# Boese0601/Dyadic-Interaction-Modeling

Hardware: AMD Instinct MI355X
Metric: listener clips/sec (T=300, EMOCA-56) (higher is better)
Workload: dtype bf16; 1 GPU; C3: B=256/GPU synthetic dyad clips, T=300, SLMFT.forward(mode='val'): listener VQ encode + encoder + 299-step AR decode (top-k 52 sampling) + VQ decode; global_batch=256, seq_len=300, gather=tokens+coeffs, gather_bytes_per_rank=17452032

## Files before the change

### dyadic-interaction-modeling_amd/build.py

```python
import concurrent.futures
import os
import subprocess
import sys

HERE = os.path.dirname(os.path.abspath(__file__))
CSRC = os.path.join(HERE, "csrc")
OBJ = os.path.join(CSRC, "_obj")
LIB = os.path.join(HERE, "libdimx_hip.so")
SOURCES = ["gemm.hip", "gemm_x3.hip", "gemm256.hip", "norm.hip", "attention.hip", "attention_tr.hip", "mlp_fused.hip", "decode_attn.hip", "vq.hip", "elementwise.hip", "kv_prefill.hip", "chain.hip", "model.hip", "generate.hip", "ops.hip", "stream_attn.hip", "win_attn.hip", "stream.hip",
           "train_kernels.hip", "train_attn.hip", "train_vq.hip", "train.hip", "lstm.hip", "train_lstm.hip", "train_spk.hip", "fd_select.hip", "mesh_metrics.hip",
           "listener_metrics.hip", "kmeans_sid.hip", "seq_score.hip", "beam.hip", "consensus.hip", "retrieval.hip", "decode_attn_kv8.hip"]
HEADERS = ["common.hpp", "model.hpp", "stages.hpp", "train.hpp", "decode_attn_body.hpp", "sample_pick.hpp", "online_softmax_body.hpp", "frechet.hpp", "pick_gather.hpp", os.path.join("..", "..", "include", "dimx.h")]
FLAGS = ["--offload-arch=gfx950", "-O3", "-std=c++17", "-fPIC", "-Wall", "-Wno-unused-function",
         "-Wno-unused-variable", "-ffp-contract=on"]
SRC_FLAGS = {"attention_tr.hip": ["-fno-slp-vectorize"]}


def _hipcc():
    for c in (os.environ.get("HIPCC"), "/opt/rocm/bin/hipcc", "hipcc"):
        if c and (os.path.isabs(c) and os.path.exists(c) or not os.path.isabs(c)):
            return c
    return "hipcc"


def _file_hash(paths, extra=""):
    import hashlib
    hsh = hashlib.sha256(extra.encode())
    for f in paths:
        with open(f, "rb") as fh:
            hsh.update(os.path.basename(f).encode() + b"\0" + fh.read())
    return hsh.hexdigest()


def _compile(src):
    obj = os.path.join(OBJ, src.replace(".hip", ".o"))
    deps = [os.path.join(CSRC, src)] + [os.path.join(CSRC, h) for h in HEADERS]
    flags = FLAGS + SRC_FLAGS.get(src, [])
    want = _file_hash(deps, " ".join(flags))
    stamp = obj + ".srchash"
    if os.path.exists(obj) and os.path.exists(stamp):
        with open(stamp) as fh:
            if fh.read().strip() == want:
                return obj, False
    tmp = "%s.tmp.%d" % (obj, os.getpid())
    cmd = [_hipcc()] + flags + ["-c", os.path.join(CSRC, src), "-o", tmp]
    r = subprocess.run(cmd, capture_output=True, text=True)
    if r.returncode != 0:
        if os.path.exists(tmp):
            os.remove(tmp)
        raise RuntimeError("hipcc failed for %s:\n%s\n%s" % (src, r.stdout, r.stderr))
    if r.stderr.strip():
        sys.stderr.write(r.stderr)
    os.replace(tmp, obj)
    with open(stamp, "w") as fh:
        fh.write(want + "\n")
    return obj, True


def have_hipcc():
    import shutil
    c = _hipcc()
    return (os.path.isabs(c) and os.path.exists(c)) or shutil.which(c) is not None


STAMP = LIB + ".srchash"


def _src_hash():
    import hashlib
    hsh = hashlib.sha256((" ".join(FLAGS) + repr(sorted(SRC_FLAGS.items()))).encode())
    for f in SOURCES + HEADERS:
        with open(os.path.join(CSRC, f), "rb") as fh:
            hsh.update(f.encode() + b"\0" + fh.read())
    return hsh.hexdigest()


def stale():
    if not (os.path.exists(LIB) and os.path.exists(STAMP)):
        return True
    with open(STAMP) as fh:
        return fh.read().strip() != _src_hash()


def build(force=False):
    import fcntl
    os.makedirs(OBJ, exist_ok=True)
    with open(os.path.join(OBJ, ".lock"), "w") as lock:
        fcntl.flock(lock, fcntl.LOCK_EX)
        try:
            if not force and not stale():
                return LIB
            if force:
                for f in os.listdir(OBJ):
                    if f != ".lock" and os.path.isfile(os.path.join(OBJ, f)):
                        os.remove(os.path.join(OBJ, f))
            with concurrent.futures.ThreadPoolExecutor(max_workers=min(8, len(SOURCES))) as ex:
                res = list(ex.map(_compile, SOURCES))
            objs = [o for o, _ in res]
# ... 18 lines not shown
```

### dyadic-interaction-modeling_amd/csrc/common.hpp

```cpp
#pragma once
#include <hip/hip_runtime.h>
#include <stdint.h>
#include <stdio.h>
#include <string.h>
#include <string>

#include "../../include/dimx.h"

namespace dimx {

void set_error(const char* fmt, ...);
const char* get_error();

#define DIMX_HIP(expr)                                                                       \
    do {                                                                                     \
        hipError_t _e = (expr);                                                              \
        if (_e != hipSuccess) {                                                              \
            dimx::set_error("%s:%d: %s -> %s", __FILE__, __LINE__, #expr, hipGetErrorString(_e)); \
            return DIMX_ERR_HIP;                                                             \
        }                                                                                    \
    } while (0)

#define DIMX_REQUIRE(cond, code, ...)       \
    do {                                    \
// ... 193 lines not shown
    int kloop;
    int M, N, K;
    int conv_T;
    const int32_t* conv_lens;
    int conv_C;
    const float* bias;
    int act;
    const float* residual;
    int ldr;
    const float* rowadd;
    int rowadd_mode;
    float rowadd_scale;
    int rowadd_off, ld_rowadd;
    int rowadd_div;
    int rowT;
    OutSeg seg[3];
    int nseg, seg_width;
    int allow_splitk;
    int splitk;
    int force_simple;
    int cfg;
    int force_splitk;
    int out_slabs;
    long slab_stride;
    int stage_out;
    const float* ln_stats;
    const float* ln_colsum;
    int ln_C;
    unsigned* ln_err;
    int w_tiled;
    const void* w3;
    long w3_plane;
    int x3_decode;
    int vt_pack4;
};

void gemm_args_init(GemmArgs& a);
void gemm_set_plain_out(GemmArgs& a, void* C, int ldc);
int launch_gemm(const GemmArgs& a, hipStream_t s);
bool gemm256_eligible(const GemmArgs& a);
int launch_gemm256(const GemmArgs& a, hipStream_t s);
int launch_gemm256_segs(const GemmArgs& a, const OutSeg* segs, int nseg, int seg_width, hipStream_t s);
bool gemm_use_x3(const GemmArgs& a);
bool gemm_x3_plan(const GemmArgs& a, int* bn_out, int* sp_out);
int launch_gemm_x3(const GemmArgs& a, hipStream_t s);
int launch_split_x3(const float* w, void* planes, size_t n, hipStream_t s);
int gemm_plan_splits(const GemmArgs& a);

int launch_layernorm(int out_dtype, const float* x, void* y, const float* gamma, const float* beta, int M,
                     int C, hipStream_t s);
int launch_add_slabs_layernorm(int out_dtype, float* x, const float* slabs, int nslab, long slab_stride, void* y,
                               const float* gamma, int M, int C, hipStream_t s);
int launch_instnorm(int out_dtype, const float* x, void* y, const int32_t* lens, int B, int T, int C,
                    hipStream_t s);

struct AttnArgs {
    int dtype;
    const void *q, *k, *vt;
    void* o;
    long q_sb, q_st, q_sh;
    long k_sb, k_st, k_sh;
    long v_sb, v_sh, v_sd;
    int v_rows;
    long v_st;
    long o_sb, o_st, o_sh;
    int B, H, Lq, Lk, D;
    float scale;
    int causal;
    const int32_t* lens;
    const uint8_t* kmask;
    int kmask_ld;
    unsigned long long* kwords;
    size_t kwords_cap;
    int kwords_ready;
};
int launch_pack_key_words(const uint8_t* kmask, int kmask_ld, const int32_t* lens, int B, int Lk, unsigned long long* words, size_t cap,
                          hipStream_t s);
int launch_attention(const AttnArgs& a, hipStream_t s);
int launch_attention_tr(const AttnArgs& a, hipStream_t s);
size_t mlp_fused_packed_bytes(int C, int F);
int mlp_fused_pack(const float* w1, const float* b1, const float* w2, int C, int F, uint16_t* out);
int launch_mlp_fused(float* x, const void* packed, const float* b2, const float* ln_g, const float* ln_b, int M, int C, int F, int act,
                     hipStream_t s);

struct DecodeAttnArgs {
    int dtype;
    const void* q;
    int q_ld;
    int q_f32;
    int nslab;
    long slab_stride;
    int force_nsplit;
    int rows_per_clip;
    const void* knew;
    const void* vnew;
    int kv_ld;
    void* kcache;
    void* vcache;
    int Tmax;
    void* out;
    int o_ld;
    int B, H;
    const int32_t* step;
    int n_keys;
    const uint8_t* kmask;
    int kmask_ld;
    float scale;
    const void* tab;
    int tab_ld, tab_koff, tab_voff, tab_rows;
    const int32_t* hist;
    int hist_ld;
    int win, lookahead;
};
int launch_decode_attn(const DecodeAttnArgs& a, hipStream_t s);

struct Kv8AttnArgs {
    const float* q;
    int q_ld, nslab;
    long slab_stride;
    const uint8_t* kcodes;
    const float* kscale;
    const uint8_t* vcodes;
    const float* vscale;
    int Tmax;
    void* out;
    int out_dtype, o_ld;
    int B, H;
    int n_keys;
    const uint8_t* kmask;
    int kmask_ld;
    float scale;
    int force_nsplit;
    int win, lookahead;
    const int32_t* step;
};
int launch_decode_attn_kv8(const Kv8AttnArgs& a, hipStream_t s);
int launch_kv8_quant(int dtype, const void* cache, int B, int H, int Tp, int T, uint8_t* codes, float* scales, hipStream_t s);

int launch_vq_argmin(const float* z, int N, const float* Et , const float* ee ,
                     int32_t* idx, float* best_d, float* margin, hipStream_t s);

struct ChainGemmDesc {
    const void* W;
    int N, K, ldw;
    int cols, rows_pad, ncb, nkt;
};
struct ChainArgs {
    int B;
    ChainGemmDesc g1;
    const void* A1;
    int lda1;
    float* xr;
    float* x;
    int C;
    const float* slabs;
    int nslab;
    long slab_stride;
    void* y;
    const float* gamma;
    ChainGemmDesc g2;
    float* out2;
    int ld_out2;
    unsigned* counters;
    unsigned* seen;
    const int32_t* step;
    unsigned* err;
// ... 196 lines not shown
```

### dyadic-interaction-modeling_amd/csrc/generate.hip

```cpp
#include <stdlib.h>

#include "stages.hpp"

namespace dimx {

static void chain_desc(ChainGemmDesc& d, const Linear& L) { d.W = L.w; d.N = L.N; d.K = L.K; d.ldw = L.Kp; }

static bool gen_use_chain(dimx_handle h, int B, int S) {
    if (!h->use_chain || h->at != DIMX_BF16 || S != 1 || h->gen_groups > 1 || !h->chain_err_dev) return false;
    const DecGeom& dg = h->decg;
    ChainArgs c;
    memset(&c, 0, sizeof(c));
    c.B = B;
    c.C = dg.dim;
    const XAttn& sa = h->dec.self_[0];
    const XAttn& ca = h->dec.cross[0];
    chain_desc(c.g1, sa.out);
    c.lda1 = dg.heads * dg.dim_head;
    chain_desc(c.g2, ca.qkv);
    if (!chain_supported(c, h->cu_count)) return false;
    chain_desc(c.g2, h->dec.logits);
    c.g1.W = nullptr;
    return chain_supported(c, h->cu_count) && 3 * dg.depth + 1 <= kChainSites;
}
// ... 1007 lines not shown
                       const uint8_t* ctx_mask, const int32_t* lens, int B, int T, int beam_width, int32_t* tokens, double* scores,
                       int32_t* backptr, float* logits_out, void* beam_state, size_t beam_state_bytes, int flags, void* ws, size_t ws_bytes,
                       void* stream) {
    DIMX_REQUIRE(h, DIMX_ERR_ARG, "null handle");
    DIMX_NO_SESSION(h, "generate_beam");
    DIMX_REQUIRE(h->variant == 0, DIMX_ERR_ARG, "generate_beam: beam search is implemented for variant 0 (SLMFT) only; this handle is variant %d",
                 h->variant);
    DIMX_REQUIRE(!h->xwin_on, DIMX_ERR_ARG, "generate_beam: not available while the cross-attention window is on (dimx_set_cross_lookahead)");
    DIMX_REQUIRE(beam_width_supported(beam_width), DIMX_ERR_ARG, "generate_beam: beam_width %d not in {1,2,4,5,8,10}", beam_width);
    DIMX_REQUIRE(prompt && scores && T >= 2 && Pmax >= 1 && Pmax <= T - 1 && ld_prompt >= Pmax, DIMX_ERR_ARG,
                 "generate_beam: need scores, 1 <= Pmax <= T - 1 and ld_prompt >= Pmax (Pmax=%d T=%d ld_prompt=%d)", Pmax, T, ld_prompt);
    DIMX_REQUIRE(P0 >= 1 && P0 <= Pmax, DIMX_ERR_ARG, "generate_beam: need 1 <= P0 <= Pmax (P0=%d Pmax=%d)", P0, Pmax);
    DIMX_REQUIRE((flags & ~1) == 0, DIMX_ERR_ARG, "generate_beam: unknown flags 0x%x", flags);
    DIMX_REQUIRE(B >= 1 && T <= h->d.max_seq_len, DIMX_ERR_ARG, "B=%d T=%d out of range (T <= %d)", B, T, h->d.max_seq_len);
    const size_t R = (size_t)B * beam_width;
    DIMX_REQUIRE(beam_state && ((uintptr_t)beam_state % 8) == 0 && beam_state_bytes >= DIMX_BEAM_STATE_BYTES(B, beam_width), DIMX_ERR_ARG,
                 "generate_beam: the beam state needs %zu bytes, 8-byte aligned (DIMX_BEAM_STATE_BYTES); got %zu", (size_t)DIMX_BEAM_STATE_BYTES(B, beam_width),
                 beam_state_bytes);
    const int p0 = (flags & 1) ? 1 : P0;
    DIMX_REQUIRE(p0 == 1 || h->decg.dim_head == 64, DIMX_ERR_ARG, "generate_beam: the prefill needs 64-wide heads");
    const size_t need = workspace_bytes_prompt(h, B, T, beam_width, p0);
    DIMX_REQUIRE(ws_bytes >= need, DIMX_ERR_WORKSPACE, "generate_beam: workspace %zu < required %zu (dimx_workspace_bytes_prompt)", ws_bytes, need);
    BeamCall bm;
    bm.cum = (double*)beam_state;
    bm.parent = (int32_t*)((double*)beam_state + R);
    bm.backptr = backptr;
    bm.lens = lens;
    const GenRequest q{{prompt, ld_prompt, Pmax, prompt_len, p0 - 1}, ctx_mask, B, T, beam_width, 0.f, 0, nullptr, 0,
                       tokens, logits_out, ws, ws_bytes, (hipStream_t)stream, &bm};
    DIMX_TRY(generate_checked(h, q));
    DIMX_HIP(hipMemcpyAsync(scores, bm.cum, R * sizeof(double), hipMemcpyDeviceToDevice, (hipStream_t)stream));
    return DIMX_OK;
}

int dimx_set_sampler_filter(dimx_handle h, int kind, float a, float b) {
    DIMX_REQUIRE(h, DIMX_ERR_ARG, "null handle");
    DIMX_TRY(check_sampler_filter(kind, a, b));
    h->filter_kind = kind;
    h->filter_a = kind == DIMX_FILTER_TOP_K ? 0.f : a;
    h->filter_b = kind == DIMX_FILTER_TOP_A ? b : 0.f;
    return DIMX_OK;
}

int dimx_set_cross_lookahead(dimx_handle h, int on, int lookahead) {
    DIMX_REQUIRE(h, DIMX_ERR_ARG, "null handle");
    DIMX_NO_SESSION(h, "set_cross_lookahead");
    DIMX_REQUIRE(h->variant == 0, DIMX_ERR_ARG, "set_cross_lookahead: online generation is implemented for variant 0 (SLMFT) only; this handle is variant %d",
                 h->variant);
    h->xwin_on = on ? 1 : 0;
    h->xwin_lookahead = on ? lookahead : 0;
    return DIMX_OK;
}

int dimx_cross_lookahead(dimx_handle h, int* on, int* lookahead) {
    DIMX_REQUIRE(h, DIMX_ERR_ARG, "null handle");
    if (on) *on = h->xwin_on;
    if (lookahead) *lookahead = h->xwin_lookahead;
    return DIMX_OK;
}

size_t dimx_cross_kv8_bytes(dimx_handle h, int B, int T) { return kv8_bytes(h, B, T); }

int dimx_set_cross_kv8(dimx_handle h, void* buf, size_t bytes) {
    DIMX_REQUIRE(h, DIMX_ERR_ARG, "null handle");
    DIMX_NO_SESSION(h, "set_cross_kv8");
    DIMX_REQUIRE(h->variant == 0, DIMX_ERR_ARG, "set_cross_kv8: FP8 cross K/V is implemented for variant 0 (SLMFT) only; this handle is variant %d",
                 h->variant);
    DIMX_REQUIRE(buf == nullptr || (h->decg.dim_head == 64 && (uintptr_t)buf % 256 == 0), DIMX_ERR_ARG,
                 "set_cross_kv8: the buffer must be 256-byte aligned and the decoder's heads 64 wide");
    h->kv8_buf = buf;
    h->kv8_bytes = buf ? bytes : 0;
    return DIMX_OK;
}

int dimx_cross_kv8(dimx_handle h, void** buf, size_t* bytes) {
    DIMX_REQUIRE(h, DIMX_ERR_ARG, "null handle");
    if (buf) *buf = h->kv8_buf;
    if (bytes) *bytes = h->kv8_bytes;
    return DIMX_OK;
}

int dimx_chain_faults(dimx_handle h) { return h ? h->chain_faults : 0; }
int dimx_qkv0_table_builds(dimx_handle h) { return h ? h->qkv0_builds : 0; }
int dimx_kv0_table_generations(dimx_handle h) { return h ? h->kv0_generations : 0; }
int dimx_sample_head_generations(dimx_handle h) { return h ? h->sample_head_generations : 0; }

int dimx_debug_chain_fault(dimx_handle h, int n_calls) {
    DIMX_REQUIRE(h && n_calls >= 0, DIMX_ERR_ARG, "debug_chain_fault: bad argument");
    h->chain_fault_inject = n_calls;
    h->graph_valid = false;
    return DIMX_OK;
}

}
```

### dyadic-interaction-modeling_amd/csrc/model.hip

```cpp
#include <stdarg.h>
#include <stdlib.h>
#include <set>

#include "stages.hpp"

namespace dimx {

static thread_local char g_err[1024] = "";
void set_error(const char* fmt, ...) {
    va_list ap;
    va_start(ap, fmt);
    vsnprintf(g_err, sizeof(g_err), fmt, ap);
    va_end(ap);
}
const char* get_error() { return g_err; }

static std::string vq_prefix(int which) { return which == 0 ? "speaker_vq." : "listener_vq."; }

struct KeySpec {
    std::string name;
    std::vector<int64_t> shape;
};

static void vq_keys(const dimx_dims& d, int which, std::vector<KeySpec>& out) {
// ... 232 lines not shown
        }
        row += rows;
    }
    void* p;
    if (c->at == DIMX_BF16) {
        std::vector<uint16_t> wb(w.size());
        for (size_t i = 0; i < w.size(); ++i) wb[i] = host_f32_to_bf16(w[i]);
        DIMX_TRY(dev_upload(c, wb.data(), wb.size() * 2, &p));
    } else {
        DIMX_TRY(dev_upload(c, w.data(), w.size() * 4, &p));
    }
    out->w = p;
    out->N = N;
    out->K = K;
    out->Kp = Kp;
    out->bias = nullptr;
    if (!bias.empty()) DIMX_TRY(upload_f32(c, bias, &out->bias));
    return DIMX_OK;
}

static int make_x3(dimx_ctx* c, Linear* L) {
    static const bool off = getenv("DIMX_NO_X3") != nullptr;
    L->w3 = nullptr;
    if (off || c->at != DIMX_F32 || !L->w || L->Kp % 32 != 0) return DIMX_OK;
    const size_t n = (size_t)L->N * L->Kp;
    void* p = nullptr;
    DIMX_HIP(hipMalloc(&p, 3 * n * 2));
    c->dev_allocs.push_back(p);
    DIMX_TRY(launch_split_x3((const float*)L->w, p, n, nullptr));
    DIMX_HIP(hipStreamSynchronize(nullptr));
    L->w3 = p;
    return DIMX_OK;
}

static int pack_linear_scaled(dimx_ctx* c, const std::string& wname, const std::string& gname, const std::string& bias,
                              Linear* out, const float** colsum) {
    auto wi = c->host.find(wname), gi = c->host.find(gname);
    DIMX_REQUIRE(wi != c->host.end() && gi != c->host.end(), DIMX_ERR_WEIGHT, "missing weight %s / %s", wname.c_str(), gname.c_str());
    const int N = (int)wi->second.shape[0], K = (int)wi->second.shape[1];
    DIMX_REQUIRE((int)gi->second.data.size() == K && K % 64 == 0, DIMX_ERR_WEIGHT, "%s: gamma / K mismatch", wname.c_str());
    std::vector<uint16_t> wb((size_t)N * K);
    std::vector<float> cs(N);
    for (int n = 0; n < N; ++n) {
        double acc = 0.0;
        for (int k = 0; k < K; ++k) {
            const uint16_t b = host_f32_to_bf16(wi->second.data[(size_t)n * K + k] * gi->second.data[k]);
            wb[(size_t)n * K + k] = b;
            const uint32_t u = (uint32_t)b << 16;
            float f;
            memcpy(&f, &u, 4);
            acc += f;
        }
        cs[n] = (float)acc;
    }
    void *p, *q;
    DIMX_TRY(dev_upload(c, wb.data(), wb.size() * 2, &p));
    DIMX_TRY(dev_upload(c, cs.data(), cs.size() * 4, &q));
    out->w = p;
    out->N = N;
    out->K = K;
    out->Kp = K;
    out->bias = nullptr;
    if (!bias.empty()) DIMX_TRY(upload_f32(c, bias, &out->bias));
    *colsum = (const float*)q;
    return DIMX_OK;
}

static int pack_mlp(dimx_ctx* c, const std::string& w1, const std::string& b1, const std::string& w2, const void** out) {
    *out = nullptr;
    if (c->at != DIMX_BF16) return DIMX_OK;
    auto i1 = c->host.find(w1), ib = c->host.find(b1), i2 = c->host.find(w2);
    DIMX_REQUIRE(i1 != c->host.end() && ib != c->host.end() && i2 != c->host.end(), DIMX_ERR_WEIGHT, "missing weight %s", w1.c_str());
    const int F = (int)i1->second.shape[0], C = (int)i1->second.shape[1];
    const size_t bytes = mlp_fused_packed_bytes(C, F);
    if (bytes == 0 || (int)i2->second.shape[0] != C || (int)i2->second.shape[1] != F) return DIMX_OK;
    std::vector<uint16_t> img(bytes / 2);
    DIMX_TRY(mlp_fused_pack(i1->second.data.data(), ib->second.data.data(), i2->second.data.data(), C, F, img.data()));
    void* p;
    DIMX_TRY(dev_upload(c, img.data(), bytes, &p));
    *out = p;
    return DIMX_OK;
}

static int pack_vq(dimx_ctx* c, int which) {
    VQNet& v = c->vq[which];
    const VQGeom& vg = c->vqg[which];
    const std::string p = vq_prefix(which), e = p + "encoder.", d = p + "decoder.";
    DIMX_TRY(pack_linear(c, {e + "vertice_mapping.0.weight"}, e + "vertice_mapping.0.bias", false, &v.vm));
    DIMX_TRY(pack_linear(c, {e + "squasher.0.0.weight"}, e + "squasher.0.0.bias", true, &v.conv));
    DIMX_TRY(pack_linear(c, {e + "encoder_linear_embedding.net.weight"}, e + "encoder_linear_embedding.net.bias", false, &v.le));
    DIMX_TRY(pack_linear(c, {e + "encoder_linear_embedding_post.net.weight"}, e + "encoder_linear_embedding_post.net.bias", false, &v.post));
    if (vg.has_decoder) {
        DIMX_TRY(pack_linear(c, {d + "decoder_linear_embedding_pre.net.weight"}, d + "decoder_linear_embedding_pre.net.bias", false, &v.pre));
        DIMX_TRY(pack_linear(c, {d + "expander.0.0.weight"}, d + "expander.0.0.bias", true, &v.dconv));
        DIMX_TRY(pack_linear(c, {d + "decoder_linear_embedding.net.weight"}, d + "decoder_linear_embedding.net.bias", false, &v.dle));
        DIMX_TRY(pack_linear(c, {d + "vertice_map_reverse.weight"}, "", false, &v.rev));
    }
    for (int s = 0; s < (vg.has_decoder ? 2 : 1); ++s) {
        const std::string pre = s == 0 ? e + "encoder_transformer." : d + "decoder_transformer.";
        VQBlock* blk = s == 0 ? v.enc : v.dec;
        for (int i = 0; i < vg.layers; ++i) {
            const std::string a = pre + "net." + std::to_string(2 * i) + ".fn.";
            const std::string m = pre + "net." + std::to_string(2 * i + 1) + ".fn.";
            DIMX_TRY(upload_f32(c, a + "norm.weight", &blk[i].ln1_g));
            DIMX_TRY(upload_f32(c, a + "norm.bias", &blk[i].ln1_b));
            DIMX_TRY(pack_linear(c, {a + "fn.to_qkv.weight"}, "", false, &blk[i].qkv));
            DIMX_TRY(pack_linear(c, {a + "fn.to_out.weight"}, a + "fn.to_out.bias", false, &blk[i].out));
            DIMX_TRY(upload_f32(c, m + "norm.weight", &blk[i].ln2_g));
            DIMX_TRY(upload_f32(c, m + "norm.bias", &blk[i].ln2_b));
            DIMX_TRY(pack_linear(c, {m + "fn.l1.weight"}, m + "fn.l1.bias", false, &blk[i].l1));
            DIMX_TRY(pack_linear(c, {m + "fn.l2.weight"}, m + "fn.l2.bias", false, &blk[i].l2));
            DIMX_TRY(pack_mlp(c, m + "fn.l1.weight", m + "fn.l1.bias", m + "fn.l2.weight", &blk[i].mlp));
        }
    }
    DIMX_TRY(upload_f32(c, e + "encoder_pos_embedding.pe", &v.pe_enc));
    if (vg.has_decoder) DIMX_TRY(upload_f32(c, d + "decoder_pos_embedding.pe", &v.pe_dec));
    DIMX_TRY(upload_f32(c, p + "quantize.embedding.weight", &v.E));
    const HostTensor& E = c->host[p + "quantize.embedding.weight"];
    const int ne = vg.n_embed, zd = vg.zdim;
    std::vector<float> Et((size_t)zd * ne), ee(ne);
    for (int j = 0; j < ne; ++j) {
        float s = 0.f;
        for (int k = 0; k < zd; ++k) {
            const float x = E.data[(size_t)j * zd + k];
            Et[(size_t)k * ne + j] = x;
            s = fmaf(x, x, s);
        }
        ee[j] = s;
    }
    void* pp;
    DIMX_TRY(dev_upload(c, Et.data(), Et.size() * 4, &pp));
    v.Et = (const float*)pp;
    DIMX_TRY(dev_upload(c, ee.data(), ee.size() * 4, &pp));
    v.ee = (const float*)pp;
    return DIMX_OK;
}

static int pack_xattn(dimx_ctx* c, const std::string& p, bool cross, XAttn* a) {
    DIMX_TRY(upload_f32(c, p + "0.0.weight", &a->ln_g));
    if (cross) {
        DIMX_TRY(pack_linear(c, {p + "1.to_q.weight"}, "", false, &a->qkv));
    } else {
        DIMX_TRY(pack_linear(c, {p + "1.to_q.weight", p + "1.to_k.weight", p + "1.to_v.weight"}, "", false, &a->qkv));
    }
    DIMX_TRY(pack_linear(c, {p + "1.to_out.weight"}, "", false, &a->out));
    return DIMX_OK;
}
static int pack_xff(dimx_ctx* c, const std::string& p, XFF* f) {
    DIMX_TRY(upload_f32(c, p + "0.0.weight", &f->ln_g));
    DIMX_TRY(pack_linear(c, {p + "1.ff.0.0.weight"}, p + "1.ff.0.0.bias", false, &f->f1));
    DIMX_TRY(pack_linear(c, {p + "1.ff.2.weight"}, p + "1.ff.2.bias", false, &f->f2));
    DIMX_TRY(pack_mlp(c, p + "1.ff.0.0.weight", p + "1.ff.0.0.bias", p + "1.ff.2.weight", &f->mlp));
    return DIMX_OK;
}
static int pack_xenc(dimx_ctx* c, const std::string& pre, XEnc* e) {
    DIMX_TRY(pack_linear(c, {pre + "project_in.weight"}, c->host.count(pre + "project_in.bias") ? pre + "project_in.bias" : "", false,
                         &e->proj_in));
    DIMX_TRY(upload_f32(c, pre + "pos_emb.emb.weight", &e->pos_emb));
    for (int i = 0; i < c->encg[0].depth; ++i) {
        DIMX_TRY(pack_xattn(c, xl(pre, 2 * i), false, &e->attn[i]));
        DIMX_TRY(pack_xff(c, xl(pre, 2 * i + 1), &e->ff[i]));
    }
    DIMX_TRY(upload_f32(c, pre + "attn_layers.final_norm.weight", &e->final_g));
    return DIMX_OK;
}

static void free_packed(dimx_ctx* c) {
    for (void* p : c->dev_allocs) (void)hipFree(p);
    c->dev_allocs.clear();
    c->packed_mask = 0;
    ++c->dec_epoch;
}


static std::vector<KeySpec> comp_keys(const dimx_dims& d, int comp) {
    std::vector<KeySpec> k;
    if (comp == COMP_MESH) {
        mesh_keys(d, k);
        return k;
    }
    if (d.variant == 1) {
        if (comp == COMP_VQ0) legacy_speaker_vq_keys(d, k);
        if (comp == COMP_VQ1) vq_keys(d, 1, k);
        if (comp == COMP_ENC) xenc_keys(d, "generator.encoder.", (int64_t)d.spk_face_quan_num * d.vq_zdim, k);
        if (comp == COMP_DEC) {
            xdec_keys(d, "generator.decoder.net.", k);
            k.push_back({"generator.decoder.net.pos_emb.emb.weight", {d.max_seq_len, d.dim + d.dim_a}});
        }
        return k;
    }
    if (comp == COMP_VQ0) vq_keys(d, 0, k);
    if (comp == COMP_VQ1) vq_keys(d, 1, k);
    if (comp == COMP_ENC) {
        xenc_keys(d, "encoder_s.", d.dim_in, k);
        xenc_keys(d, "encoder_joint.", d.dim, k);
        k.push_back({"patch_embed_s", {1, 1, d.dim_in}});
        k.push_back({"patch_embed_dec_s", {1, 1, d.dim}});
        k.push_back({"norm_s.weight", {d.dim}});
        k.push_back({"norm_s.bias", {d.dim}});
        if (d.variant == 2) slm_extra_keys(d, k, 1);
    }
    if (comp == COMP_DEC) {
        xdec_keys(d, "decoder_joint.net.", k);
        if (d.variant == 2) slm_extra_keys(d, k, 2);
    }
    return k;
}

static int ensure_packed(dimx_ctx* c, int need) {
    if ((c->packed_mask & need) == need) return DIMX_OK;
    DIMX_HIP(hipSetDevice(c->device));
    for (int comp = 1; comp <= COMP_MESH; comp <<= 1) {
        if (!(need & comp) || (c->packed_mask & comp)) continue;
        int missing = 0;
        std::string first;
        for (const auto& k : comp_keys(c->d, comp))
            if (!c->host.count(k.name)) {
                if (!missing) first = k.name;
                ++missing;
            }
        DIMX_REQUIRE(missing == 0, DIMX_ERR_WEIGHT, "%d weights of this stage not loaded (first: %s)", missing,
                     first.c_str());
        if (comp == COMP_VQ0) DIMX_TRY(pack_vq(c, 0));
        if (comp == COMP_VQ1) DIMX_TRY(pack_vq(c, 1));
        if (comp == COMP_ENC && c->variant == 1) {
            DIMX_TRY(pack_xenc(c, "generator.encoder.", &c->enc_s));
// ... 108 lines not shown
    return at == DIMX_BF16 && D <= 64;
}

static void set_qkv_out(GemmArgs& g, void* q, void* k, void* vt, int T, int H, int D, int Tp, bool rowv = false) {
    const int segw = H * D;
    g.rowT = T;
    g.nseg = 3;
    g.seg_width = segw;
    for (int i = 0; i < (rowv ? 3 : 2); ++i) {
        g.seg[i].ptr = i == 0 ? q : (i == 1 ? k : vt);
        g.seg[i].sb = (long)T * segw;
        g.seg[i].st = segw;
        g.seg[i].sh = D;
        g.seg[i].sd = 1;
        g.seg[i].D = D;
    }
    if (rowv) return;
    g.seg[2].ptr = vt;
    g.seg[2].sb = (long)H * D * Tp;
    g.seg[2].sh = (long)D * Tp;
    g.seg[2].sd = Tp;
    g.seg[2].st = 1;
    g.seg[2].D = D;
}

void set_attn_packed(AttnArgs& a, int dtype, const void* q, const void* k, const void* vt, void* o, int B,
                            int H, int Lq, int Lk, int D, int Tp_k, bool rowv) {
    memset(&a, 0, sizeof(a));
    const int segw = H * D;
    a.dtype = dtype;
    a.q = q;
    a.k = k;
    a.vt = vt;
    a.o = o;
    a.q_sb = (long)Lq * segw;
    a.q_st = segw;
    a.q_sh = D;
    a.k_sb = (long)Lk * segw;
    a.k_st = segw;
    a.k_sh = D;
    a.v_sb = (long)H * D * Tp_k;
    a.v_sh = (long)D * Tp_k;
    a.v_sd = Tp_k;
    if (rowv) {
        a.v_rows = 1;
        a.v_sb = (long)Lk * segw;
        a.v_st = segw;
        a.v_sh = D;
    }
    a.o_sb = (long)Lq * segw;
    a.o_st = segw;
    a.o_sh = D;
    a.B = B;
    a.H = H;
    a.Lq = Lq;
    a.Lk = Lk;
    a.D = D;
}


int linear(const dimx_ctx* c, const void* A, int lda, const Linear& L, int M, int out_dtype, void* out, int ldo, hipStream_t st, int act,
           const float* residual) {
    GemmArgs g;
    gemm_lin(c, A, lda, L, M, g);
    g.out_dtype = out_dtype; g.act = act;
    g.residual = residual; g.ldr = residual ? ldo : 0;
    gemm_set_plain_out(g, out, ldo);
    return launch_gemm(g, st);
}
int residual_linear(const dimx_ctx* c, const void* A, int lda, const Linear& L, int M, float* h, int ld, hipStream_t st) {
    return linear(c, A, lda, L, M, DIMX_F32, h, ld, st, ACT_NONE, h);
}

constexpr int kFusedMlpMinRows = 8192;

int ff_sublayer(const dimx_ctx* c, const BlockBufs& b, const float* ln_g, const float* ln_b, const Linear& f1,
                       const Linear& f2, const void* mlp, int act, int M, int C, hipStream_t st) {
    if (mlp && M >= kFusedMlpMinRows) return launch_mlp_fused(b.h, mlp, f2.bias, ln_g, ln_b, M, C, f1.N, act, st);
    DIMX_TRY(launch_layernorm(c->at, b.h, b.y, ln_g, ln_b, M, C, st));
    DIMX_TRY(linear(c, b.y, C, f1, M, c->at, b.f, f1.N, st, act));
    return residual_linear(c, b.f, f1.N, f2, M, b.h, C, st);
}

int self_attn_qkv(const dimx_ctx* c, const BlockBufs& b, const float* ln_g, const float* ln_b, const Linear& qkv, int B,
                         int T, int C, int heads, int D, AttnArgs& a, hipStream_t st) {
    const bool rowv = qkv_row_v(c->at, D);
    DIMX_TRY(launch_layernorm(c->at, b.h, b.y, ln_g, ln_b, B * T, C, st));
    GemmArgs g;
    gemm_lin(c, b.y, C, qkv, B * T, g);
    g.out_dtype = c->at;
    set_qkv_out(g, b.q, b.k, b.vt, T, heads, D, tpad(T), rowv);
    DIMX_TRY(launch_gemm(g, st));
    set_attn_packed(a, c->at, b.q, b.k, b.vt, b.o, B, heads, T, T, D, tpad(T), rowv);
    return DIMX_OK;
}

int attn_out(const dimx_ctx* c, const BlockBufs& b, AttnArgs& a, const Linear& out, int C, hipStream_t st) {
    a.kwords = b.kw; a.kwords_cap = b.kw_cap;
    DIMX_TRY(launch_attention(a, st));
    return residual_linear(c, b.o, a.H * a.D, out, a.B * a.Lq, b.h, C, st);
}

int cross_attn_sublayer(const dimx_ctx* c, const BlockBufs& b, const XAttn& x, AttnArgs& a, const uint8_t* ctx_mask, int C,
                               hipStream_t st, const float* v_rows) {
    const int M = a.B * a.Lq, Tp = tpad(a.Lk);
    DIMX_TRY(launch_layernorm(c->at, b.h, b.y, x.ln_g, nullptr, M, C, st));
    DIMX_TRY(linear(c, b.y, C, x.qkv, M, c->at, b.q, a.H * a.D, st));
    if (v_rows) DIMX_TRY(launch_kv_rows_to_vt(v_rows, Tp, (float*)a.vt, Tp, a.B, a.Lk, a.H, st));
    a.scale = 1.0f / sqrtf((float)a.D); a.kmask = ctx_mask; a.kmask_ld = a.Lk;
    return attn_out(c, b, a, x.out, C, st);
}

float* win_q_rows(const BlockBufs& b, int B, int n, int inner, size_t es) {
    const unsigned char *lo = (const unsigned char*)b.k, *hi = (const unsigned char*)b.vt + (size_t)B * inner * tpad(n) * es;
    return lo && b.vt && lo < hi && (size_t)(hi - lo) >= (size_t)B * n * inner * 4 ? (float*)b.k : nullptr;
}

struct VQScratch : BlockBufs {
    void *xa, *h1;
    float *conv, *z;
    int32_t* idx_tmp;
};

static void plan_vq(const dimx_ctx* c, const VQGeom& vg, Arena& ar, int B, int T, VQScratch& s) {
    const size_t M = (size_t)B * T, es = es_of(c);
    const int H = vg.hidden, I = vg.inter, Tp = tpad(T);
    s.xa = ar.take(M * (vg.in_pad > 128 ? vg.in_pad : 128) * es);
    s.h1 = ar.take(M * H * es);
    s.conv = (float*)ar.take(M * H * 4);
    s.y = ar.take(M * H * es);
    s.h = (float*)ar.take(M * H * 4);
    s.q = ar.take(M * H * es);
    s.k = ar.take(M * H * es);
    s.vt = ar.take((size_t)B * H * Tp * es);
    s.o = ar.take(M * H * es);
    s.f = ar.take(M * I * es);
    s.z = (float*)ar.take(M * vg.out_dim * 4);
    s.idx_tmp = (int32_t*)ar.take(M * vg.fqn * 4);
}

static int run_vq_blocks(const dimx_ctx* c, const VQGeom& vg, const VQBlock* blk, VQScratch& s, int B, int T,
                         const int32_t* lens, hipStream_t st) {
    const int M = B * T, Hd = vg.hidden, heads = vg.heads, D = Hd / heads;
    const float scale = 1.0f / sqrtf((float)Hd);
    for (int l = 0; l < vg.layers; ++l) {
        const VQBlock& b = blk[l];
        AttnArgs a;
        DIMX_TRY(self_attn_qkv(c, s, b.ln1_g, b.ln1_b, b.qkv, B, T, Hd, heads, D, a, st));
        a.scale = scale; a.lens = lens;
        DIMX_TRY(attn_out(c, s, a, b.out, Hd, st));
        DIMX_TRY(ff_sublayer(c, s, b.ln2_g, b.ln2_b, b.l1, b.l2, b.mlp, ACT_GELU_TANH, M, Hd, st));
    }
    return DIMX_OK;
}

static int run_vq_front(const dimx_ctx* c, const VQGeom& vg, const void* x_in, int ld_in, const Linear& conv,
                        const Linear& le, const float* pe, int pe_mode, int row_off, VQScratch& s, int B, int T,
                        const int32_t* lens, hipStream_t st, int row_div = 1) {
    const int M = B * T, Hd = vg.hidden;
    GemmArgs g;
    gemm_lin(c, x_in, ld_in, conv, M, g);
    g.conv_T = T;
    g.conv_lens = lens;
    g.conv_C = Hd;
    g.act = ACT_LEAKY;
    g.out_dtype = DIMX_F32;
    gemm_set_plain_out(g, s.conv, Hd);
    DIMX_TRY(launch_gemm(g, st));
    DIMX_TRY(launch_instnorm(c->at, s.conv, s.y, lens, B, T, Hd, st));
    gemm_lin(c, s.y, Hd, le, M, g);
    g.out_dtype = DIMX_F32;
    g.rowT = T;
    g.rowadd = pe;
    g.ld_rowadd = Hd;
    g.rowadd_mode = pe_mode == 0 ? 3 : 2;
    g.rowadd_off = pe_mode == 0 ? 0 : row_off;
    g.rowadd_div = row_div;
    gemm_set_plain_out(g, s.h, Hd);
    DIMX_TRY(launch_gemm(g, st));
    return DIMX_OK;
}

static int run_vq_encode(const dimx_ctx* c, int which, const float* x, const int32_t* lens, int B, int T, int pe_mode,
                         int row_off, VQScratch& s, float* z, int32_t* idx, hipStream_t st) {
    const VQGeom& vg = c->vqg[which];
    const VQNet& v = c->vq[which];
    const int M = B * T, Hd = vg.hidden;
    DIMX_TRY(launch_cast_pad(c->at, x, vg.in_dim, nullptr, s.xa, vg.in_pad, M, vg.in_dim, st));
    DIMX_TRY(linear(c, s.xa, vg.in_pad, v.vm, M, c->at, s.h1, Hd, st, ACT_LEAKY));
    DIMX_TRY(run_vq_front(c, vg, s.h1, Hd, v.conv, v.le, v.pe_enc, pe_mode, row_off, s, B, T, lens, st));
    DIMX_TRY(run_vq_blocks(c, vg, v.enc, s, B, T, lens, st));
    DIMX_TRY(launch_cast_pad(c->at, s.h, Hd, nullptr, s.y, Hd, M, Hd, st));
    DIMX_TRY(linear(c, s.y, Hd, v.post, M, DIMX_F32, z, vg.out_dim, st));
    DIMX_TRY(launch_vq_argmin(z, M * vg.fqn, v.Et, v.ee, idx, nullptr, nullptr, st));
    return DIMX_OK;
}

}

using namespace dimx;

extern "C" {

int dimx_version(void) { return 100; }
const char* dimx_last_error(void) { return get_error(); }

void dimx_legacy_dims(dimx_dims* d) {
    if (!d) return;
    dimx_default_dims(d);
    d->variant = 1;
    d->dim_in = 1024; d->dim = 512; d->dim_a = 0; d->enc_depth = 6; d->dec_depth = 6; d->heads = 8;
    d->max_seq_len = 1024;
    d->spk_in_dim = 824; d->spk_hidden = 768; d->spk_heads = 8; d->spk_inter = 1536; d->spk_face_quan_num = 8;
}

void dimx_default_dims(dimx_dims* d) {
    if (!d) return;
    memset(d, 0, sizeof(*d));
    d->vq_in_dim = 56; d->vq_hidden = 384; d->vq_layers = 6; d->vq_heads = 8; d->vq_inter = 1536;
    d->vq_n_embed = 512; d->vq_zdim = 128;
    d->dim_in = 56; d->dim = 384; d->dim_a = 768; d->enc_depth = 4; d->dec_depth = 4; d->heads = 12;
    d->dim_head = 64; d->num_tokens = 512; d->max_seq_len = 2048; d->ff_mult = 4;
}

int dimx_create(dimx_handle* h, int device_id, const dimx_dims* dims, int numeric_mode) {
    DIMX_REQUIRE(h, DIMX_ERR_ARG, "dimx_create: null handle pointer");
    DIMX_REQUIRE(numeric_mode == DIMX_MODE_PARITY_F32 || numeric_mode == DIMX_MODE_PERF_BF16, DIMX_ERR_ARG,
                 "dimx_create: numeric_mode %d", numeric_mode);
    dimx_dims d;
    dimx_default_dims(&d);
    if (dims) d = *dims;
    DIMX_REQUIRE(d.vq_hidden == 384 && d.vq_heads == 8 && d.vq_zdim == 128 && d.vq_n_embed == 512 && d.vq_in_dim == 56,
                 DIMX_ERR_ARG, "dimx_create: only the DIM-Listener VQ geometry (56/384/8/128/512) is built");
    if (d.variant == 0 || d.variant == 2) {
        DIMX_REQUIRE(d.dim == 384 && d.dim_a == 768 && d.dim_head == 64 && d.heads == 12 && d.num_tokens == 512 &&
                         d.vq_layers <= 8 && d.enc_depth <= 8 && d.dec_depth <= 8 && d.max_seq_len <= 2048,
                     DIMX_ERR_ARG, "dimx_create: only the SLMFT geometry (384+768, 12x64, 512 tokens) is built");
    } else {
        DIMX_REQUIRE(d.variant == 1 && d.dim == 512 && d.dim_a == 0 && d.dim_head == 64 && d.heads == 8 &&
                         d.num_tokens == 512 && d.enc_depth <= 8 && d.dec_depth <= 8 && d.max_seq_len <= 2048 &&
                         d.spk_hidden == 768 && d.spk_heads == 8 && d.spk_in_dim == 824 && d.spk_face_quan_num == 8,
                     DIMX_ERR_ARG, "dimx_create: only the legacy ListenerGenerator geometry (824/768 VQ, 512, 8x64) is built");
    }
    DIMX_REQUIRE(d.mesh_dim == 0 || (d.variant == 2 && d.mesh_dim > 0), DIMX_ERR_ARG,
                 "dimx_create: the mesh head (mesh_dim %d) belongs to a handle of variant 2", d.mesh_dim);
    int ndev = 0;
    DIMX_HIP(hipGetDeviceCount(&ndev));
    DIMX_REQUIRE(device_id >= 0 && device_id < ndev, DIMX_ERR_ARG, "dimx_create: device %d of %d", device_id, ndev);
    DIMX_HIP(hipSetDevice(device_id));
    dimx_ctx* c = new dimx_ctx();
    c->device = device_id;
    c->d = d;
    c->mode = numeric_mode;
    c->at = numeric_mode == DIMX_MODE_PERF_BF16 ? DIMX_BF16 : DIMX_F32;
    c->variant = d.variant;
    const VQGeom lvq = {d.vq_in_dim, 64, d.vq_hidden, d.vq_heads, d.vq_inter, d.vq_layers, d.vq_zdim, 1, d.vq_zdim,
                        d.vq_n_embed, true};
    c->vqg[0] = c->vqg[1] = lvq;
    if (d.variant == 1) {
        c->vqg[0] = {d.spk_in_dim, (d.spk_in_dim + 63) / 64 * 64, d.spk_hidden, d.spk_heads, d.spk_inter, d.vq_layers,
                     d.spk_face_quan_num * d.vq_zdim, d.spk_face_quan_num, d.vq_zdim, d.vq_n_embed, false};
        const int din = d.spk_face_quan_num * d.vq_zdim;
        c->encg[0] = c->encg[1] = {din, din, d.dim, d.heads, d.dim_head, d.enc_depth, d.ff_mult, 0};
        c->decg = {d.dim, d.heads, d.dim_head, d.dec_depth, d.ff_mult, 1, d.num_tokens, d.dim};
    } else {
        const int causal = d.variant == 2 ? 0 : 1, abs_pos = d.variant == 2 ? 1 : 0;
        c->encg[0] = {d.dim_in, 64, d.dim, d.heads, d.dim_head, d.enc_depth, d.ff_mult, causal};
        c->encg[1] = {d.dim, d.dim, d.dim, d.heads, d.dim_head, d.enc_depth, d.ff_mult, causal};
        c->decg = {d.dim + d.dim_a, d.heads, d.dim_head, d.dec_depth, d.ff_mult, abs_pos, d.num_tokens, d.dim + d.dim_a};
    }
    for (const auto& k : all_keys(d)) c->required.push_back(k.name);
    const char* ng = getenv("DIMX_NO_GRAPH");
    c->use_graph = (ng && ng[0] == '1') ? 0 : 1;
    const char* nc = getenv("DIMX_NO_CHAIN");
    c->use_chain = (nc && nc[0] == '1') ? 0 : 1;
    c->use_layer_chain = getenv("DIMX_NO_LAYER_CHAIN") ? 0 : 1;
    c->multi_tr = getenv("DIMX_NO_MULTI_TR") ? 0 : 1;
    c->use_qkv0_table = getenv("DIMX_NO_QKV0_TABLE") ? 0 : 1;
    c->use_kv0_table = getenv("DIMX_NO_KV0_TABLE") ? 0 : 1;
    c->use_sample_head = getenv("DIMX_NO_SAMPLE_HEAD") ? 0 : 1;
    if (getenv("DIMX_LAYER_PROF")) {
        void* p = nullptr;
        if (hipMalloc(&p, (size_t)8 * 256 * 16 * 8) == hipSuccess) {
            (void)hipMemset(p, 0, (size_t)8 * 256 * 16 * 8);
            c->layer_prof_dev = (unsigned long long*)p;
        }
    }
    if (const char* pg = getenv("DIMX_PREFILL_GROUPS")) {
        const int v = atoi(pg);
        if (v >= 1 && v <= dimx_ctx::kPreGroups) c->prefill_groups = v;
    }
    {
        int cus = 0;
        if (hipDeviceGetAttribute(&cus, hipDeviceAttributeMultiprocessorCount, device_id) == hipSuccess) c->cu_count = cus;
    }
    const char* gg = getenv("DIMX_GEN_GROUPS");
    if (gg && atoi(gg) >= 1 && atoi(gg) <= dimx_ctx::kMaxGroups) c->gen_groups = atoi(gg);
    *h = c;
    return DIMX_OK;
}

int dimx_destroy(dimx_handle h) {
    if (!h) return DIMX_OK;
    (void)hipSetDevice(h->device);
    for (int g = 0; g < dimx_ctx::kMaxGroups; ++g) {
        if (h->graph_multi[g]) (void)hipGraphExecDestroy(h->graph_multi[g]);
        if (h->graph_exec[g]) (void)hipGraphExecDestroy(h->graph_exec[g]);
        if (h->grp_stream[g]) (void)hipStreamDestroy(h->grp_stream[g]);
        if (h->ev_join[g]) (void)hipEventDestroy(h->ev_join[g]);
    }
    if (h->ev_fork) (void)hipEventDestroy(h->ev_fork);
    for (int g = 0; g < dimx_ctx::kPreGroups - 1; ++g) {
        if (h->pre_stream[g]) (void)hipStreamDestroy(h->pre_stream[g]);
        if (h->pre_join[g]) (void)hipEventDestroy(h->pre_join[g]);
    }
    if (h->pre_fork) (void)hipEventDestroy(h->pre_fork);
    if (h->cap_stream) (void)hipStreamDestroy(h->cap_stream);
    if (h->chain_err_ev) (void)hipEventDestroy(h->chain_err_ev);
    if (h->chain_err_dev) (void)hipFree(h->chain_err_dev);
    if (h->chain_stats_dev) (void)hipFree(h->chain_stats_dev);
    if (h->layer_prof_dev) (void)hipFree(h->layer_prof_dev);
    if (h->qkv0_table) (void)hipFree(h->qkv0_table);
    if (h->kv0_image) (void)hipFree(h->kv0_image);
    if (h->chain_err_host) (void)hipHostFree(h->chain_err_host);
    free_packed(h);
    stream_forget(h);
    train_forget(h);
    delete h;
    return DIMX_OK;
}

int dimx_numeric_mode(dimx_handle h) { return h ? h->mode : DIMX_ERR_ARG; }

int dimx_set_shard(dimx_handle h, int row_offset, int rows_total) {
    DIMX_REQUIRE(h, DIMX_ERR_ARG, "set_shard: null handle");
    DIMX_REQUIRE(row_offset >= 0 && (rows_total == 0 || rows_total > row_offset), DIMX_ERR_ARG,
                 "set_shard: row_offset %d, rows_total %d", row_offset, rows_total);
    h->shard_row_off = row_offset;
    h->shard_rows_total = rows_total;
    return DIMX_OK;
}

int dimx_begin_checkpoint(dimx_handle h) {
    DIMX_REQUIRE(h, DIMX_ERR_ARG, "dimx_begin_checkpoint: null handle");
    std::set<std::string> spec;
    for (const auto& k : all_keys(h->d)) spec.insert(k.name);
    bool dirty = false;
    for (auto it = h->host.begin(); it != h->host.end();) {
        if (!spec.count(it->first)) {
            it = h->host.erase(it);
            dirty = true;
        } else {
            ++it;
        }
    }
    if (dirty) {
        (void)hipSetDevice(h->device);
        (void)hipDeviceSynchronize();
        free_packed(h);
        h->graph_valid = false;
        h->ctx_ready = false;
    }
    return DIMX_OK;
// ... 192 lines not shown
    s.xj = ar.take((size_t)B * 2 * T * c->encg[0].dim * es);
    s.m2 = (uint8_t*)ar.take((size_t)B * 2 * T);
}

static size_t workspace_bytes(const dimx_ctx* c, int B, int T, int S = 1) {
    Arena p(nullptr, 0);
    CtxPersist cp;
    plan_persist(c, p, B, T, cp);
    const size_t persist = align_up(p.off, 256);
    size_t scratch = 0;
    for (int w = 0; w < 2; ++w) {
        Arena a(nullptr, 0);
        VQScratch s;
        plan_vq(c, c->vqg[w], a, B, T, s);
        scratch = a.off > scratch ? a.off : scratch;
    }
    {
        Arena a(nullptr, 0);
        EncScratch s;
        plan_enc(c, a, B, T, s);
        if (c->variant == 0) a.take((size_t)B * T * c->decg.ctx_dim * es_of(c));
        if (c->variant == 1) {
            VQScratch v;
            plan_vq(c, c->vqg[0], a, B, T, v);
            a.take((size_t)B * 4);
        }
        scratch = a.off > scratch ? a.off : scratch;
    }
    if (c->variant == 2) {
        Arena a(nullptr, 0);
        SlmScratch s;
        plan_slm(c, a, B, T, s);
        scratch = a.off > scratch ? a.off : scratch;
    }
    if (c->d.mesh_dim > 0) {
        Arena a(nullptr, 0);
        MeshScratch s;
        plan_mesh(c, a, B, T, s);
        scratch = a.off > scratch ? a.off : scratch;
    }
    if (T >= 2) {
        Arena a(nullptr, 0);
        DecScratch s;
        plan_dec(c, a, B, T, s);
        scratch = a.off > scratch ? a.off : scratch;
        Arena g(nullptr, 0);
        GenScratch gs;
        plan_gen(c, g, B * S, T, gs);
        scratch = g.off > scratch ? g.off : scratch;
    }
    return persist + align_up(scratch, 256) + 4096 + 65536;
}

size_t workspace_bytes_prompt(const dimx_ctx* c, int B, int T, int S, int P0) {
    const size_t base = workspace_bytes(c, B, T, S);
    if (P0 <= 1 || T < 2) return base;
    Arena p(nullptr, 0);
    CtxPersist cp;
    plan_persist(c, p, B, T, cp);
    Arena g(nullptr, 0);
    GenScratch gs;
    plan_gen(c, g, B * S, T, gs);
    PrefillScratch ps;
    plan_prefill(c, g, B, P0 - 1, T, ps);
    const size_t need = align_up(p.off, 256) + align_up(g.off, 256) + 4096 + 65536;
    return need > base ? need : base;
}

static int run_xenc(const dimx_ctx* c, const EncGeom& eg, const XEnc& e, const void* x_in, int ld_in, EncScratch& s,
                    int B, int T, const uint8_t* mask, int out_dtype, void* out, hipStream_t st) {
    const int M = B * T, dim = eg.dim, heads = eg.heads, D = eg.dim_head;
    GemmArgs g;
    gemm_lin(c, x_in, ld_in, e.proj_in, M, g);
    g.out_dtype = DIMX_F32;
    g.rowT = T;
    g.rowadd = e.pos_emb;
    g.ld_rowadd = dim;
    g.rowadd_mode = 1;
    g.rowadd_scale = 1.0f / sqrtf((float)dim);
    gemm_set_plain_out(g, s.h, dim);
    DIMX_TRY(launch_gemm(g, st));
    for (int l = 0; l < eg.depth; ++l) {
        AttnArgs a;
        DIMX_TRY(self_attn_qkv(c, s, e.attn[l].ln_g, nullptr, e.attn[l].qkv, B, T, dim, heads, D, a, st));
        a.scale = 1.0f / sqrtf((float)D); a.causal = eg.causal; a.kmask = mask; a.kmask_ld = T;
        DIMX_TRY(attn_out(c, s, a, e.attn[l].out, dim, st));
        DIMX_TRY(ff_sublayer(c, s, e.ff[l].ln_g, nullptr, e.ff[l].f1, e.ff[l].f2, e.ff[l].mlp, ACT_GELU_ERF, M, dim, st));
    }
    DIMX_TRY(launch_layernorm(out_dtype, s.h, out, e.final_g, nullptr, M, dim, st));
    return DIMX_OK;
}

int check_common(dimx_handle h, int B, int T, void* ws, size_t ws_bytes, int need, int S) {
    DIMX_REQUIRE(h, DIMX_ERR_ARG, "null handle");
    DIMX_REQUIRE(B >= 1 && T >= 1 && T <= h->d.max_seq_len, DIMX_ERR_ARG, "B=%d T=%d out of range (T <= %d)", B, T,
                 h->d.max_seq_len);
    DIMX_REQUIRE(ws && ((uintptr_t)ws % 256) == 0, DIMX_ERR_ARG, "workspace must be 256-byte aligned");
    const size_t need_bytes = workspace_bytes(h, B, T, S);
    DIMX_REQUIRE(ws_bytes >= need_bytes, DIMX_ERR_WORKSPACE, "workspace %zu < required %zu", ws_bytes, need_bytes);
    DIMX_HIP(hipSetDevice(h->device));
    DIMX_TRY(ensure_packed(h, need));
    return DIMX_OK;
}

int project_cross_kv(dimx_handle h, const void* ctx, const CtxPersist& cp, int B, int T, int for_generate,
                     hipStream_t st);
int legacy_encode_ctx(dimx_handle h, const float* v_speaker, const uint8_t* mask, int B, int T, int for_generate,
                      float* enc_out, float* x_speaker_out, int32_t* idx_out, void* ws, size_t ws_bytes,
                      hipStream_t st);

struct ClipGroups {
    int G;
    int b0[dimx_ctx::kPreGroups + 1];
    hipStream_t st[dimx_ctx::kPreGroups];
};
static int clip_groups_fork(dimx_handle h, int B, int T, hipStream_t st, ClipGroups& cg, bool one_group = false) {
    int G = one_group ? 1 : h->prefill_groups;
    if (G == 0) {
        const size_t rows = (size_t)B * T;
        G = rows > 196608 ? 1 : rows >= 32768 ? 4 : rows >= 16384 ? 2 : 1;
    }
    if (G > B) G = B;
    cg.G = G;
    for (int g = 0; g <= G; ++g) cg.b0[g] = (int)((long)B * g / G);
    cg.st[0] = st;
    if (G == 1) return DIMX_OK;
    {
        hipStreamCaptureStatus cs = hipStreamCaptureStatusNone;
        if (hipStreamIsCapturing(st, &cs) != hipSuccess || cs != hipStreamCaptureStatusNone) {
            (void)hipGetLastError();
            cg.G = 1;
            cg.b0[1] = B;
            return DIMX_OK;
        }
        if (hipStreamQuery(st) != hipSuccess) (void)hipStreamSynchronize(st);
        (void)hipGetLastError();
    }
    if (!h->pre_fork) DIMX_HIP(hipEventCreateWithFlags(&h->pre_fork, hipEventDisableTiming));
    DIMX_HIP(hipEventRecord(h->pre_fork, st));
    for (int g = 1; g < G; ++g) {
        if (!h->pre_stream[g - 1]) DIMX_HIP(hipStreamCreateWithFlags(&h->pre_stream[g - 1], hipStreamNonBlocking));
        if (!h->pre_join[g - 1]) DIMX_HIP(hipEventCreateWithFlags(&h->pre_join[g - 1], hipEventDisableTiming));
        cg.st[g] = h->pre_stream[g - 1];
        DIMX_HIP(hipStreamWaitEvent(cg.st[g], h->pre_fork, 0));
    }
    return DIMX_OK;
}
static int clip_groups_join(dimx_handle h, const ClipGroups& cg) {
    hipError_t bad = hipSuccess;
    for (int g = 1; g < cg.G; ++g) {
        hipError_t e = hipEventRecord(h->pre_join[g - 1], cg.st[g]);
        if (e == hipSuccess) e = hipStreamWaitEvent(cg.st[0], h->pre_join[g - 1], 0);
        if (e != hipSuccess) {
            (void)hipStreamSynchronize(cg.st[g]);
            bad = e;
        }
    }
    DIMX_HIP(bad);
    return DIMX_OK;
}

static int clip_groups_close(dimx_handle h, const ClipGroups& cg, int rc) {
    const int jrc = clip_groups_join(h, cg);
    return rc != DIMX_OK ? rc : jrc;
}

Arena scratch_arena(const dimx_ctx* c, void* ws, size_t ws_bytes, int B, int T, CtxPersist* cp) {
// ... 497 lines not shown
```

### dyadic-interaction-modeling_amd/csrc/model.hpp

```cpp
#pragma once
#include <map>
#include <string>
#include <vector>

#include "common.hpp"

namespace dimx {

struct Linear {
    void* w = nullptr;
    const float* bias = nullptr;
    int N = 0, K = 0, Kp = 0;
    void* w3 = nullptr;
};

struct VQBlock {
    const float *ln1_g, *ln1_b, *ln2_g, *ln2_b;
    Linear qkv, out, l1, l2;
    const void* mlp = nullptr;
};

struct VQNet {
    Linear vm, conv, le, post;
    VQBlock enc[8];
    Linear pre, dconv, dle, rev;
    VQBlock dec[8];
    const float* pe_enc = nullptr;
    const float* pe_dec = nullptr;
    const float* E = nullptr;
    const float* Et = nullptr;
    const float* ee = nullptr;
};

struct XAttn {
    const float* ln_g;
    Linear qkv;
    Linear kv;
    Linear out;
    Linear q_ln;
    const float* q_ln_colsum = nullptr;
};
struct XFF {
    const float* ln_g;
    Linear f1, f2;
    Linear f1_ln;
    const float* f1_ln_colsum = nullptr;
    const void* mlp = nullptr;
};
struct XEnc {
    Linear proj_in;
    const float* pos_emb = nullptr;
    XAttn attn[8];
    XFF ff[8];
    const float* final_g = nullptr;
};
struct XDec {
    const float* tok_emb = nullptr;
    const float* pos_emb = nullptr;
    XAttn self_[8], cross[8];
    XFF ff[8];
    const float* final_g = nullptr;
    Linear logits;
    Linear cross_kv_all;
};

struct MeshHead {
    const float *w_ih[2][2], *w_hh[2][2], *b_ih[2][2], *b_hh[2][2];
    Linear l1, l2;
};

struct VQGeom {
    int in_dim, in_pad, hidden, heads, inter, layers, out_dim, fqn, zdim, n_embed;
    bool has_decoder;
};
struct EncGeom {
    int dim_in, in_pad, dim, heads, dim_head, depth, ff_mult, causal;
};
struct DecGeom {
    int dim, heads, dim_head, depth, ff_mult, abs_pos, num_tokens, ctx_dim;
};

struct HostTensor {
    std::vector<float> data;
    std::vector<int64_t> shape;
};

struct Arena {
    unsigned char* base;
    size_t off;
    size_t cap;
    bool overflow;
    Arena(void* b, size_t c) : base((unsigned char*)b), off(0), cap(c), overflow(false) {}
    void* take(size_t bytes) {
        off = align_up(off, 256);
        void* p = base ? base + off : nullptr;
        off += bytes;
        if (base && off > cap) overflow = true;
        return p;
    }
};

struct BeamCall {
    double* cum = nullptr;
    int32_t* parent = nullptr;
    int32_t* backptr = nullptr;
    const int32_t* lens = nullptr;
    bool operator==(const BeamCall& o) const { return cum == o.cum && parent == o.parent && backptr == o.backptr && lens == o.lens; }
};

struct StepRoute {
    bool chain = false;
    bool defer = false;
    bool layer_kernel[8] = {};
    bool logits_chain = false;
    bool multi_tr = false;
    bool win = false;
    int lookahead = 0;
    bool kv8 = false;
    const float* qkv0 = nullptr;
// ... 19 lines not shown
    int filter_kind;
    BeamCall beam;
    int xwin_on, xwin_lookahead;
    bool guided;
    const void* branch_out;
    const void* kv8;
    bool operator==(const GraphKey& o) const {
        return ws == o.ws && B == o.B && T == o.T && top_k == o.top_k && noise == o.noise && start == o.start && mask == o.mask &&
               tokens == o.tokens && logits_out == o.logits_out && G == o.G && S == o.S && chain == o.chain && defer == o.defer &&
               logits_chain == o.logits_chain && multi_tr == o.multi_tr && fault_inject == o.fault_inject &&
               layer_kernel == o.layer_kernel && qkv0 == o.qkv0 && kv0 == o.kv0 && sample_head == o.sample_head && prompt_len == o.prompt_len &&
               ld_prompt == o.ld_prompt && Pmax == o.Pmax && filter_kind == o.filter_kind && beam == o.beam && xwin_on == o.xwin_on &&
               xwin_lookahead == o.xwin_lookahead && guided == o.guided && branch_out == o.branch_out && kv8 == o.kv8;
    }
};

}

namespace dimx {
int vq_pe_buffers(dimx_ctx* c, int which, const float** pe_enc, const float** pe_dec);
void train_forget(dimx_ctx* h);
void stream_forget(dimx_ctx* h);
}

struct dimx_ctx {
    int device = 0;
    dimx_dims d;
    int variant = 0;
    dimx::VQGeom vqg[2];
    dimx::EncGeom encg[2];
    dimx::DecGeom decg;
    int mode = 0;
    int at = DIMX_F32;
    std::map<std::string, dimx::HostTensor> host;
    std::vector<std::string> required;
    int packed_mask = 0;
    std::vector<void*> dev_allocs;
    dimx::VQNet vq[2];
    dimx::XEnc enc_s, enc_joint, enc_l;
    dimx::XDec dec;
    const float *patch_s = nullptr, *patch_dec_s = nullptr, *norm_s_g = nullptr, *norm_s_b = nullptr;
    const float *patch_l = nullptr, *patch_dec_l = nullptr, *norm_l_g = nullptr, *norm_l_b = nullptr;
    const float *norm_j_g = nullptr, *norm_j_b = nullptr;
    bool ctx_ready = false;
    int ctx_B = 0, ctx_T = 0, ctx_for_generate = 0;
    void* ctx_ws = nullptr;
    static constexpr int kMaxGroups = 8;
    hipGraphExec_t graph_exec[kMaxGroups] = {};
    hipGraphExec_t graph_multi[kMaxGroups] = {};
    int graph_unroll = 16;
    static constexpr int kPreGroups = 4;
    int prefill_groups = 0;
    hipStream_t pre_stream[kPreGroups - 1] = {};
    hipEvent_t pre_fork = nullptr, pre_join[kPreGroups - 1] = {};
    hipStream_t grp_stream[kMaxGroups] = {};
    hipEvent_t ev_fork = nullptr, ev_join[kMaxGroups] = {};
    int gen_groups = 1;
    hipStream_t cap_stream = nullptr;
    dimx::GraphKey graph_key{};
    bool graph_valid = false;
    int use_graph = 1;
    int use_chain = 1;
    int cu_count = 0;
    float* chain_stats_dev = nullptr;
    int defer_ln = 1;
    unsigned long long* layer_prof_dev = nullptr;
    int multi_tr = 1;
    int use_layer_chain = 1;
    unsigned* chain_err_dev = nullptr;
    unsigned* chain_err_host = nullptr;
    hipEvent_t chain_err_ev = nullptr;
    int chain_faults = 0;
    int chain_fault_inject = 0;
    int use_qkv0_table = 1;
    float* qkv0_table = nullptr;
    int qkv0_M = 0, qkv0_at = -1;
    uint64_t qkv0_epoch = 0;
    uint64_t dec_epoch = 1;
    int qkv0_builds = 0;
    int use_kv0_table = 1;
    void* kv0_image = nullptr;
    int kv0_generations = 0;
    int use_sample_head = 1;
    int sample_head_generations = 0;
    int shard_row_off = 0, shard_rows_total = 0;
    int filter_kind = 0;
    float filter_a = 0.f, filter_b = 0.f;
    int xwin_on = 0, xwin_lookahead = 0;
    void* kv8_buf = nullptr;
    size_t kv8_bytes = 0;
    int twin_on = 0, twin_lookahead = 0;
    const uint8_t* tcond_keep = nullptr;
    void* stream_sess = nullptr;
    dimx::MeshHead mesh;
    int lstm_faults = 0;
    int spk_embed_rows = 0;
};
```

### dyadic-interaction-modeling_amd/csrc/ops.hip

```cpp
#include "stages.hpp"

using namespace dimx;

extern "C" {

int dimx_op_lstm_layer(int dtype, const float* x, int B, int T, int In, int H, const float* const* w_ih, const float* const* w_hh,
                       const float* const* b_ih, const float* const* b_hh, float* y, int flags, int* faults_out, void* stream) {
    DIMX_REQUIRE(dtype == DIMX_F32, DIMX_ERR_ARG, "lstm_layer: only the f32 recurrence is built (dtype %d)", dtype);
    DIMX_REQUIRE(B >= 1 && T >= 1 && In >= 4, DIMX_ERR_ARG, "lstm_layer: bad shape");
    hipStream_t st = (hipStream_t)stream;
    int dev = 0, cus = 0;
    DIMX_HIP(hipGetDevice(&dev));
    DIMX_HIP(hipDeviceGetAttribute(&cus, hipDeviceAttributeMultiprocessorCount, dev));
    const size_t bytes = lstm_scratch_bytes(B, T, In);
    void* scratch = nullptr;
    DIMX_HIP(hipMalloc(&scratch, bytes));
    int faults = 0;
    const int rc = lstm_layer_run(x, B, T, In, H, w_ih, w_hh, b_ih, b_hh, y, scratch, bytes, flags, cus, &faults, st);
    const hipError_t e = hipStreamSynchronize(st);
    (void)hipFree(scratch);
    if (faults_out) *faults_out = faults;
    DIMX_TRY(rc);
    DIMX_HIP(e);
    return DIMX_OK;
// ... 362 lines not shown
                           void* vcache, void* out, int o_ld, int B, int H, int Tmax, const int32_t* step_dev, int n_keys,
                           const uint8_t* kmask, int kmask_ld, int rows_per_clip, float scale, int nsplit, void* stream) {
    return op_decode_attn_ex(dtype, q, q_ld, q_is_f32, nslab, slab_stride, self_attn, kcache, vcache, out, o_ld, B, H, Tmax, step_dev, n_keys,
                             kmask, kmask_ld, rows_per_clip, scale, nsplit, 0, 0, stream);
}

int dimx_op_decode_attn_tab(int dtype, const void* q, int q_ld, int q_is_f32, int nslab, long slab_stride, void* kcache, void* vcache,
                            void* out, int o_ld, int B, int H, int Tmax, const int32_t* step_dev, float scale, int nsplit, const void* tab,
                            int tab_ld, int tab_koff, int tab_voff, int tab_rows, const int32_t* hist, int hist_ld, void* stream) {
    const OpTabArgs t = {tab, tab_ld, tab_koff, tab_voff, tab_rows, hist, hist_ld};
    return op_decode_attn_ex(dtype, q, q_ld, q_is_f32, nslab, slab_stride, 1, kcache, vcache, out, o_ld, B, H, Tmax, step_dev, 0, nullptr, 0,
                             1, scale, nsplit, 0, 0, stream, &t);
}

int dimx_op_decode_attn_win(int dtype, const void* q, int q_ld, int q_is_f32, int nslab, long slab_stride, void* kcache, void* vcache,
                            void* out, int o_ld, int B, int H, int Tmax, const int32_t* step_dev, int n_keys, const uint8_t* kmask,
                            int kmask_ld, int rows_per_clip, float scale, int nsplit, int lookahead, void* stream) {
    DIMX_REQUIRE(step_dev != nullptr, DIMX_ERR_ARG, "op_decode_attn_win: the windowed form needs a step counter");
    return op_decode_attn_ex(dtype, q, q_ld, q_is_f32, nslab, slab_stride, 0, kcache, vcache, out, o_ld, B, H, Tmax, step_dev, n_keys, kmask,
                             kmask_ld, rows_per_clip, scale, nsplit, 1, lookahead, stream);
}

int dimx_op_kv8_quantize(int dtype, const void* cache, int B, int H, int Tp, int T, uint8_t* codes, float* scales, void* stream) {
    return launch_kv8_quant(dtype, cache, B, H, Tp, T, codes, scales, (hipStream_t)stream);
}

int dimx_op_decode_attn_kv8(int out_dtype, const void* q, int q_ld, int q_is_f32, int nslab, long slab_stride, const uint8_t* kcodes,
                            const float* kscale, const uint8_t* vcodes, const float* vscale, void* out, int o_ld, int B, int H, int Tmax,
                            const int32_t* step_dev, int n_keys, const uint8_t* kmask, int kmask_ld, int rows_per_clip, float scale, int nsplit,
                            int lookahead, int win, void* stream) {
    DIMX_REQUIRE(q_is_f32, DIMX_ERR_ARG, "op_decode_attn_kv8: q must be f32 split-K slabs");
    DIMX_REQUIRE(rows_per_clip <= 1, DIMX_ERR_ARG, "op_decode_attn_kv8: one row per clip (rows_per_clip = %d)", rows_per_clip);
    DIMX_REQUIRE(!win || step_dev != nullptr, DIMX_ERR_ARG, "op_decode_attn_kv8: the windowed form needs a step counter");
    Kv8AttnArgs a;
    memset(&a, 0, sizeof(a));
    a.q = (const float*)q; a.q_ld = q_ld; a.nslab = nslab; a.slab_stride = slab_stride;
    a.kcodes = kcodes; a.kscale = kscale; a.vcodes = vcodes; a.vscale = vscale; a.Tmax = Tmax;
    a.out = out; a.out_dtype = out_dtype; a.o_ld = o_ld; a.B = B; a.H = H;
    a.n_keys = n_keys; a.kmask = kmask; a.kmask_ld = kmask_ld; a.scale = scale; a.force_nsplit = nsplit;
    if (win) { a.win = 1; a.lookahead = lookahead; a.step = step_dev; }
    return launch_decode_attn_kv8(a, (hipStream_t)stream);
}

int dimx_op_cross_attn_win(int dtype, const float* q, int ld, const void* kcache, const void* vcache, int Tp, void* out, int o_ld, int B, int H,
                           int Lq, int t0, int n_keys, int lookahead, const uint8_t* kmask, int kmask_ld, float scale, void* stream) {
    WinAttnArgs a;
    memset(&a, 0, sizeof(a));
    a.dtype = dtype;
    a.q = q; a.ld = ld;
    a.kcache = kcache; a.vcache = vcache; a.Tp = Tp;
    a.out = out; a.o_ld = o_ld;
    a.B = B; a.H = H; a.Lq = Lq; a.t0 = t0; a.n_keys = n_keys; a.lookahead = lookahead;
    a.kmask = kmask; a.kmask_ld = kmask_ld;
    a.scale = scale;
    return launch_win_attn(a, (hipStream_t)stream);
}

size_t dimx_mlp_fused_packed_bytes(int C, int F) { return mlp_fused_packed_bytes(C, F); }

int dimx_mlp_fused_pack(const float* w1_host, const float* b1_host, const float* w2_host, int C, int F, void* out_host, size_t out_bytes) {
    DIMX_REQUIRE(w1_host && w2_host && out_host, DIMX_ERR_ARG, "mlp_fused_pack: null argument");
    DIMX_REQUIRE(mlp_fused_packed_bytes(C, F) > 0 && out_bytes >= mlp_fused_packed_bytes(C, F), DIMX_ERR_ARG,
                 "mlp_fused_pack: C = %d F = %d unsupported or the output buffer is too small", C, F);
    return mlp_fused_pack(w1_host, b1_host, w2_host, C, F, (uint16_t*)out_host);
}

int dimx_op_mlp_fused_packed(float* x, const void* packed, const float* b2, const float* ln_g, const float* ln_b, int M, int C, int F, int act,
                             void* stream) {
    return launch_mlp_fused(x, packed, b2, ln_g, ln_b, M, C, F, act, (hipStream_t)stream);
}

int dimx_op_mlp_fused(float* x, const float* w1_host, const float* b1_host, const float* w2_host, const float* b2, const float* ln_g,
                      const float* ln_b, int M, int C, int F, int act, void* stream) {
    DIMX_REQUIRE(x && w1_host && w2_host && b2 && ln_g && M > 0, DIMX_ERR_ARG, "op_mlp_fused: null argument");
    const size_t bytes = mlp_fused_packed_bytes(C, F);
    DIMX_REQUIRE(bytes > 0, DIMX_ERR_ARG, "op_mlp_fused: C = %d F = %d not supported", C, F);
    std::vector<uint16_t> img(bytes / 2);
    DIMX_TRY(mlp_fused_pack(w1_host, b1_host, w2_host, C, F, img.data()));
    void* p = nullptr;
    DIMX_HIP(hipMalloc(&p, bytes));
    int rc = DIMX_OK;
    if (hipMemcpy(p, img.data(), bytes, hipMemcpyHostToDevice) != hipSuccess) rc = DIMX_ERR_HIP;
    if (rc == DIMX_OK) rc = launch_mlp_fused(x, p, b2, ln_g, ln_b, M, C, F, act, (hipStream_t)stream);
    if (hipStreamSynchronize((hipStream_t)stream) != hipSuccess && rc == DIMX_OK) rc = DIMX_ERR_HIP;
    (void)hipFree(p);
    return rc;
}

int dimx_op_add_slabs_layernorm(int out_dtype, float* x, const float* slabs, int nslab, long slab_stride, void* y,
                                const float* gamma, int M, int C, void* stream) {
    return launch_add_slabs_layernorm(out_dtype, x, slabs, nslab, slab_stride, y, gamma, M, C, (hipStream_t)stream);
}

int dimx_op_chain(const void* A1, int K1, const void* W1, float* x, const float* slabs, int nslab, const float* gamma,
                  void* y, const void* W2, int N2, float* out2, int B, int C, void* scratch, void* stream) {
    DIMX_REQUIRE(scratch && x && y && gamma, DIMX_ERR_ARG, "op_chain: null argument");
    int dev = 0, cus = 0;
    DIMX_HIP(hipGetDevice(&dev));
    DIMX_HIP(hipDeviceGetAttribute(&cus, hipDeviceAttributeMultiprocessorCount, dev));
    ChainArgs c;
    memset(&c, 0, sizeof(c));
    unsigned* u = (unsigned*)scratch;
    c.B = B;
    c.C = C;
    if (W1) {
        c.g1.W = W1; c.g1.N = C; c.g1.K = K1; c.g1.ldw = K1;
        c.A1 = A1; c.lda1 = K1;
        c.xr = (float*)(u + 512);
    }
    c.x = x;
    c.slabs = slabs;
    c.nslab = nslab;
    c.slab_stride = (long)B * C;
    c.y = y;
    c.gamma = gamma;
    if (W2) {
        c.g2.W = W2; c.g2.N = N2; c.g2.K = C; c.g2.ldw = C;
        c.out2 = out2; c.ld_out2 = N2;
    }
    c.counters = u;
    c.seen = u + 256;
    c.step = (const int32_t*)(u + 128);
    c.err = u + 129;
    DIMX_REQUIRE(chain_supported(c, cus), DIMX_ERR_ARG, "op_chain: shape not supported on this device (%d CUs)", cus);
    DIMX_HIP(hipMemsetAsync(u, 0, 512 * 4, (hipStream_t)stream));
    return launch_chain(c, (hipStream_t)stream);
}

int dimx_op_chain_ln(const void* A1, int K1, const void* W1, float* x, void* y, float* stats, const void* W2s,
                     const float* colsum2, int N2, float* out2, int B, int C, void* scratch, void* stream) {
    DIMX_REQUIRE(scratch && x && y && stats && A1 && W1, DIMX_ERR_ARG, "op_chain_ln: null argument");
    int dev = 0, cus = 0;
    DIMX_HIP(hipGetDevice(&dev));
    DIMX_HIP(hipDeviceGetAttribute(&cus, hipDeviceAttributeMultiprocessorCount, dev));
    ChainArgs c;
    memset(&c, 0, sizeof(c));
    unsigned* u = (unsigned*)scratch;
    c.B = B;
    c.C = C;
    c.g1.W = W1; c.g1.N = C; c.g1.K = K1; c.g1.ldw = K1;
    c.A1 = A1; c.lda1 = K1;
    c.xr = (float*)(u + 512);
    c.x = x;
    c.y = y;
    c.gamma = (const float*)x;
    c.defer = 1;
    c.stats = stats;
    if (W2s) {
        c.g2.W = W2s; c.g2.N = N2; c.g2.K = C; c.g2.ldw = C;
        c.out2 = out2; c.ld_out2 = N2;
        c.colsum2 = colsum2;
    }
    c.counters = u;
    c.seen = u + 256;
    c.step = (const int32_t*)(u + 128);
    c.err = u + 129;
    DIMX_REQUIRE(chain_supported(c, cus), DIMX_ERR_ARG, "op_chain_ln: shape not supported on this device (%d CUs)", cus);
    DIMX_HIP(hipMemsetAsync(u, 0, 512 * 4, (hipStream_t)stream));
    return launch_chain(c, (hipStream_t)stream);
}

int dimx_op_gemm_ln(int out_dtype, const void* A, const void* Ws, void* C, int M, int N, int K, const float* bias, int act,
                    const float* stats, const float* colsum, void* stream) {
    DIMX_REQUIRE(A && Ws && C && stats && colsum && M >= 1 && M <= 256, DIMX_ERR_ARG, "op_gemm_ln: bad argument");
    GemmArgs g;
    gemm_args_init(g);
// ... 149 lines not shown
```

### dyadic-interaction-modeling_amd/csrc/stages.hpp

```cpp
#pragma once
#include "model.hpp"

namespace dimx {

enum { COMP_VQ0 = 1, COMP_VQ1 = 2, COMP_ENC = 4, COMP_DEC = 8, COMP_ALL = 15, COMP_MESH = 16 };

static inline size_t es_of(const dimx_ctx* c) { return dtype_size(c->at); }
static inline int tpad(int T) { return (T + 7) / 8 * 8; }
static inline int gen_steps(const dimx_ctx* c, int T) { return c->variant == 1 ? T : T - 1; }

int gemm_lin(const dimx_ctx* c, const void* A, int lda, const Linear& L, int M, GemmArgs& g);
bool qkv_row_v(int at, int D);
void set_attn_packed(AttnArgs& a, int dtype, const void* q, const void* k, const void* vt, void* o, int B, int H, int Lq, int Lk, int D,
                     int Tp_k, bool rowv = false);

struct BlockBufs {
    float* h;
    void *y, *q, *k, *vt, *o, *f;
    unsigned long long* kw = nullptr;
    size_t kw_cap = 0;
};
int ff_sublayer(const dimx_ctx* c, const BlockBufs& b, const float* ln_g, const float* ln_b, const Linear& f1, const Linear& f2,
                const void* mlp, int act, int M, int C, hipStream_t st);
int self_attn_qkv(const dimx_ctx* c, const BlockBufs& b, const float* ln_g, const float* ln_b, const Linear& qkv, int B, int T, int C,
                  int heads, int D, AttnArgs& a, hipStream_t st);
int attn_out(const dimx_ctx* c, const BlockBufs& b, AttnArgs& a, const Linear& out, int C, hipStream_t st);
int cross_attn_sublayer(const dimx_ctx* c, const BlockBufs& b, const XAttn& x, AttnArgs& a, const uint8_t* ctx_mask, int C, hipStream_t st,
                        const float* v_rows = nullptr);

float* win_q_rows(const BlockBufs& b, int B, int n, int inner, size_t es);

struct CtxPersist {
    void* ck[8];
    void* cv[8];
};
struct GenScratch {
    void* sk[8];
    void* sv[8];
    float *x, *logits;
    void *y, *o, *f;
    float *qkv, *qc, *xr;
    long st_qkv, st_qc, st_xr, st_lg;
    int32_t* step;
    unsigned* chain_ctr;
    void* qcb;
    unsigned long long* kw;
    size_t kw_cap;
    int32_t* hist;
};
constexpr int kChainSites = 32;
constexpr int kChainSiteWords = 8 * 16 + 8 * 32;

struct GenPrompt {
    const int32_t* tok;
    int ld, Pmax;
    const int32_t* len;
    int step0;
    bool win = false;
};
struct PrefillScratch : BlockBufs {
    float* cvt;
    int32_t* inp;
};
void plan_gen(const dimx_ctx* c, Arena& ar, int B, int T, GenScratch& s);
void plan_prefill(const dimx_ctx* c, Arena& ar, int B, int n0, int T, PrefillScratch& s);
size_t workspace_bytes_prompt(const dimx_ctx* c, int B, int T, int S, int P0);
Arena scratch_arena(const dimx_ctx* c, void* ws, size_t ws_bytes, int B, int T, CtxPersist* cp);
int check_common(dimx_handle h, int B, int T, void* ws, size_t ws_bytes, int need, int S = 1);

int check_sampler_filter(int kind, float a, float b);

int linear(const dimx_ctx* c, const void* A, int lda, const Linear& L, int M, int out_dtype, void* out, int ldo, hipStream_t st,
           int act = ACT_NONE, const float* residual = nullptr);
int residual_linear(const dimx_ctx* c, const void* A, int lda, const Linear& L, int M, float* h, int ld, hipStream_t st);

constexpr int kAppendMaxRows = 16;
struct AppendAttnArgs {
    int dtype;
    const float *q, *k, *v;
    int ld;
    void *kcache, *vcache;
    int Tmax;
    void* out;
    int o_ld;
    int B, H, n0, c;
    float scale;
};
int launch_append_attn(const AppendAttnArgs& a, hipStream_t s);

struct WinAttnArgs {
    int dtype;
    const float* q;
    int ld;
    const void *kcache, *vcache;
    int Tp;
    void* out;
    int o_ld;
    int B, H, Lq, t0, n_keys, lookahead;
    const uint8_t* kmask;
    int kmask_ld;
    float scale;
};
int launch_win_attn(const WinAttnArgs& a, hipStream_t s);

struct GenRun;
struct GenSessionSpec {
    int lookahead;
    int n_keys;
// ... 14 lines not shown
```

### dyadic-interaction-modeling_amd/engine.py

```python
import ctypes

import numpy as np
import torch

from . import lib as L
from . import sampling


class Engine:
    def __init__(self, device=None, mode=L.MODE_PARITY_F32, variant="slmft", mesh_dim=0):
        if not torch.cuda.is_available():
            raise L.DimxError("dimx needs a ROCm GPU (torch.cuda.is_available() is False); "
                              "there is no CPU fallback")
        self.device = torch.device(device if device is not None else "cuda:0")
        if self.device.index is None:
            self.device = torch.device("cuda", torch.cuda.current_device())
        self.lib = L.load()
        self.mode = mode
        assert variant in ("slmft", "legacy", "slm", "speaker")
        self.variant = variant
        if variant == "speaker":
            assert mesh_dim > 0, "the speaker variant needs mesh_dim"
            self.dims = L.speaker_dims(mesh_dim)
        else:
# ... 336 lines not shown
        return out

    def _generate_prompted(self, prompt, prompt_len, prefill, no_prefill, mask_u8, T, temperature, top_k, noise, seed,
                           return_logits, n_samples, return_scores=False):
        B, Pmax = prompt.shape
        R = B * n_samples
        prompt = prompt.to(torch.int32).contiguous()
        prompt_len = prompt_len.to(torch.int32).contiguous() if prompt_len is not None else None
        window = False
        if isinstance(prefill, str) or isinstance(prefill, tuple):
            kind, prefill = (prefill, None) if isinstance(prefill, str) else prefill
            if kind != "window":
                raise ValueError("prefill=%r: an integer P0, 'window' or ('window', P0)" % (kind,))
            window = True
        P0 = int(prefill) if prefill is not None else (Pmax if prompt_len is None else 1)
        if noise is not None:
            noise = noise.to(torch.float32).contiguous()
            assert tuple(noise.shape) == (self.n_gen(T), R, self.dims.num_tokens)
        self._chk(prompt, prompt_len, mask_u8, noise)
        n = self.n_gen(T)
        tokens = torch.empty(R, n, dtype=torch.int32, device=self.device)
        lg = torch.empty(R, n, self.dims.num_tokens, dtype=torch.float32, device=self.device) if (return_logits or return_scores) else None
        ws, wsb = self.workspace(B, T, n_samples)
        L.check(self.lib.dimx_generate_prompted(self.h, L.ptr(prompt), int(prompt.stride(0)), L.ptr(prompt_len), int(Pmax), P0,
                                                L.ptr(mask_u8), B, T, int(n_samples), float(temperature), int(top_k), L.ptr(noise),
                                                int(seed) & 0xFFFFFFFFFFFFFFFF, L.ptr(tokens), L.ptr(lg),
                                                (1 if no_prefill else 0) | (2 if window else 0), ws, wsb, self._s()), "dimx_generate_prompted")
        plen = None
        if return_scores:
            no_prefill = no_prefill or (self.cross_lookahead() is not None and not window)
            plen = prompt_len.clamp(1 if no_prefill else P0, Pmax) if prompt_len is not None \
                else torch.full((B,), Pmax, dtype=torch.int32, device=self.device)
        return self._generated(tokens, lg, mask_u8, T, n_samples, plen, return_logits, return_scores)

    def generate_beam(self, start, mask_u8, T, beam_width, prompt=None, prompt_len=None, prefill=None, return_logits=False,
                      return_backptr=False):
        W = int(beam_width)
        if prompt is None:
            prompt, prompt_len, prefill = start.reshape(-1, 1), None, 1
        B, Pmax = prompt.shape
        R = B * W
        prompt = prompt.to(torch.int32).contiguous()
        prompt_len = prompt_len.to(torch.int32).contiguous() if prompt_len is not None else None
        P0 = int(prefill) if prefill is not None else (Pmax if prompt_len is None else 1)
        lens = mask_u8.sum(1, dtype=torch.int32)
        self._chk(prompt, prompt_len, mask_u8)
        n = self.n_gen(T)
        tokens = torch.empty(R, n, dtype=torch.int32, device=self.device)
        scores = torch.empty(R, dtype=torch.float64, device=self.device)
        lg = torch.empty(R, n, self.dims.num_tokens, dtype=torch.float32, device=self.device) if return_logits else None
        bp = torch.empty(R, n, dtype=torch.int32, device=self.device) if return_backptr else None
        state = torch.empty(2 * R, dtype=torch.float64, device=self.device)
        ws, wsb = self.workspace(B, T, W)
        L.check(self.lib.dimx_generate_beam(self.h, L.ptr(prompt), int(prompt.stride(0)), L.ptr(prompt_len), int(Pmax), P0,
                                            L.ptr(mask_u8), L.ptr(lens), B, T, W, L.ptr(tokens), L.ptr(scores), L.ptr(bp), L.ptr(lg),
                                            L.ptr(state), state.numel() * 8, 0, ws, wsb, self._s()), "dimx_generate_beam")
        return (tokens, scores) + ((lg,) if return_logits else ()) + ((bp,) if return_backptr else ())

    def mesh_head(self, motion, template=None, safe=False, out=None):
        B, Lq, _ = motion.shape
        V = self.dims.mesh_dim
        motion = motion.to(torch.float32).contiguous()
        template = template.to(torch.float32).contiguous() if template is not None else None
        if template is not None:
            assert tuple(template.shape) == (B, V), "template must be [B, mesh_dim]"
        if out is None:
            out = torch.empty(B, Lq, V, dtype=torch.float32, device=self.device)
        assert tuple(out.shape) == (B, Lq, V) and out.dtype == torch.float32
        self._chk(motion, template, out)
        ws, wsb = self.workspace(B, Lq)
        L.check(self.lib.dimx_mesh_head(self.h, L.ptr(motion), L.ptr(template), B, Lq, L.ptr(out), 1 if safe else 0, ws, wsb,
                                        self._s()), "dimx_mesh_head")
        return out

    def lstm_faults(self):
        return int(self.lib.dimx_lstm_faults(self.h))

    def chain_faults(self):
        return int(self.lib.dimx_chain_faults(self.h))

    def qkv0_table_builds(self):
        return int(self.lib.dimx_qkv0_table_builds(self.h))

    def kv0_table_generations(self):
        return int(self.lib.dimx_kv0_table_generations(self.h))

    def sample_head_generations(self):
        return int(self.lib.dimx_sample_head_generations(self.h))

    def debug_chain_fault(self, n_calls=1):
        L.check(self.lib.dimx_debug_chain_fault(self.h, int(n_calls)), "dimx_debug_chain_fault")


class StreamSession:

    def __init__(self, eng, B, Tmax, start, lookahead=0, temperature=1.0, top_k=52, noise=None, seed=0, prompt=None, v_speaker=None,
                 v_audio=None):
        self.eng, self.B, self.Tmax, self.lookahead = eng, int(B), int(Tmax), int(lookahead)
        self._open = False
        lib, dev = eng.lib, eng.device
        need = lib.dimx_stream_workspace_bytes(eng.h, self.B, self.Tmax)
        if need == 0:
            raise L.DimxError("dimx_stream_workspace_bytes(%d,%d) = 0: sessions need the SLMFT variant and 2 <= Tmax <= 2048" % (B, Tmax))
        self._ws = torch.empty(need + 256, dtype=torch.uint8, device=dev)
        self._V = eng.dims.num_tokens
        self._tok = torch.zeros(self.B, self.Tmax - 1, dtype=torch.int32, device=dev)
        self._lg = None
        self.begin(start, temperature, top_k, noise, seed, prompt, v_speaker, v_audio)

    def _ws_ptr(self):
        base = self._ws.data_ptr()
        aligned = (base + 255) // 256 * 256
        return ctypes.c_void_p(aligned), self._ws.numel() - (aligned - base)

    def begin(self, start=None, temperature=1.0, top_k=52, noise=None, seed=0, prompt=None, v_speaker=None, v_audio=None):
        if self._open:
            raise L.DimxError("StreamSession.begin: the session is open (end() or close() first)")
        if noise is not None:
            noise = noise.to(torch.float32).contiguous()
            assert tuple(noise.shape) == (self.Tmax - 1, self.B, self._V)
        if prompt is not None:
            return self._begin_prompted(prompt, v_speaker, v_audio, temperature, top_k, noise, seed)
        start = start.to(torch.int32).contiguous()
        self.eng._chk(start, noise)
        assert tuple(start.shape) == (self.B,)
        self._noise = noise
        self._last = (0, 0)
        ws, wsb = self._ws_ptr()
        L.check(self.eng.lib.dimx_stream_begin(self.eng.h, L.ptr(start), self.B, self.Tmax, self.lookahead, float(temperature), int(top_k),
                                               L.ptr(self._noise), int(seed) & 0xFFFFFFFFFFFFFFFF, ws, wsb, self.eng._s()),
                "dimx_stream_begin")
        self._open = True
        self.frames = 0
        self.steps = 0

    def _begin_prompted(self, prompt, v_speaker, v_audio, temperature, top_k, noise, seed):
        from . import stream as _stream
        prompt = prompt.to(torch.int32).contiguous()
        v_speaker = v_speaker.to(torch.float32).contiguous()
        v_audio = v_audio.to(torch.float32).contiguous()
        self.eng._chk(prompt, v_speaker, v_audio, noise)
        B, P = prompt.shape
        F = v_speaker.shape[1]
        assert B == self.B and v_speaker.shape[0] == B and tuple(v_audio.shape[:2]) == (B, F)
        if not _stream.prompt_fits(P, self.lookahead, F, self.Tmax):
            raise ValueError("a session cannot start from P=%d codes and F=%d frames: need 1 <= P and P + max(lookahead, 0) = %d <= F <= Tmax = %d"
                             % (P, F, P + max(self.lookahead, 0), self.Tmax))
        need = self.eng.lib.dimx_stream_workspace_bytes_prompt(self.eng.h, self.B, self.Tmax)
        if self._ws.numel() < need + 256:
            self._ws = None
            self._ws = torch.empty(need + 256, dtype=torch.uint8, device=self.eng.device)
        self._noise = noise
        ws, wsb = self._ws_ptr()
        L.check(self.eng.lib.dimx_stream_begin_prompted(self.eng.h, L.ptr(prompt), P, P, L.ptr(v_speaker), L.ptr(v_audio), F, self.B, self.Tmax,
                                                        self.lookahead, float(temperature), int(top_k), L.ptr(self._noise),
                                                        int(seed) & 0xFFFFFFFFFFFFFFFF, ws, wsb, self.eng._s()), "dimx_stream_begin_prompted")
        self._open = True
        self.frames = F
        self.steps = P - 1
        self._last = (P - 1, P - 1)
        self._tok[:, :P - 1] = prompt[:, 1:]
        if self._lg is not None:
            self._lg[:, :P - 1] = 0

    def _logits(self):
        if self._lg is None:
# ... 111 lines not shown
    a_ = a.float().contiguous()
    if planes is None:
        planes = op_split_x3(w)
    (M, K), N = a_.shape, planes.shape[1]
    flags = 4 if slabs else 0
    ns = lib.dimx_op_gemm_slabs(L.F32, M, N, K, 16 | 5) if slabs else 0
    out = torch.full((ns, M, N) if slabs else (M, N), float("nan"), dtype=torch.float32, device=a.device)
    L.check(lib.dimx_op_gemm_x3(L.ptr(a_), K, L.ptr(planes), L.ptr(out), N, M, N, K, L.ptr(bias), act, L.ptr(residual),
                                residual.shape[1] if residual is not None else 0, flags, L.stream_ptr(a.device)), "dimx_op_gemm_x3")
    return out


def op_gemm(a, w, bias=None, act=0, residual=None, bf16=False, out_bf16=False, conv_T=0, conv_lens=None,
            slabs=0, force_simple=False, cfg=0, w_tiled=False):
    lib = L.load()
    dev = a.device
    if conv_T > 0:
        N, C, _ = w.shape
        wk = w.permute(0, 2, 1).reshape(N, 5 * C)
        K = 5 * C
    else:
        wk, K = w, w.shape[1]
        N = w.shape[0]
    dt = torch.bfloat16 if bf16 else torch.float32
    a_ = a.to(dt).contiguous()
    w_ = _pad_k(wk.to(dt), 64 if bf16 else 32)
    if w_tiled:
        w_ = tile_weight(w_, 64 if bf16 else 32)
    M = a_.shape[0]
    if slabs:
        out = torch.full((slabs, M, N), float("nan"), dtype=torch.float32, device=dev)
    else:
        out = torch.empty(M, N, dtype=torch.bfloat16 if out_bf16 else torch.float32, device=dev)
    flags = (5 if slabs else 0) | (2 if force_simple else 0) | (8 if w_tiled else 0) | (cfg << 8) | (slabs << 16)
    L.check(lib.dimx_op_gemm(L.BF16 if bf16 else L.F32, L.BF16 if out_bf16 else L.F32, L.ptr(a_), a_.shape[1],
                             L.ptr(w_), w_.shape[1], L.ptr(out), N, M, N, K, L.ptr(bias), act, L.ptr(residual),
                             residual.shape[1] if residual is not None else 0, conv_T, L.ptr(conv_lens), flags,
                             L.stream_ptr(dev)), "dimx_op_gemm")
    return out


def op_lstm_layer(x, w_ih, w_hh, b_ih, b_hh, safe=False, return_faults=False):
    lib = L.load()
    dev = x.device
    B, T, In = x.shape
    H = w_hh[0].shape[1]
    x_ = x.float().contiguous()
    keep = [[t.to(dev, torch.float32).contiguous() for t in pair] for pair in (w_ih, w_hh, b_ih, b_hh)]
    arrs = [(ctypes.c_void_p * 2)(*(t.data_ptr() for t in pair)) for pair in keep]
    y = torch.empty(B, T, 2 * H, dtype=torch.float32, device=dev)
    faults = ctypes.c_int(0)
    L.check(lib.dimx_op_lstm_layer(L.F32, L.ptr(x_), B, T, In, H, arrs[0], arrs[1], arrs[2], arrs[3], L.ptr(y), 1 if safe else 0,
                                   ctypes.byref(faults), L.stream_ptr(dev)), "dimx_op_lstm_layer")
    return (y, faults.value) if return_faults else y


def op_lstm_layer_bwd(x, w_ih, w_hh, b_ih, b_hh, dy, safe=False, need_dx=True, return_faults=False):
    lib = L.load()
    dev = x.device
    B, T, In = x.shape
    H = w_hh[0].shape[1]
    x_ = x.float().contiguous()
    dy_ = dy.to(dev, torch.float32).contiguous()
    keep = [[t.to(dev, torch.float32).contiguous() for t in pair] for pair in (w_ih, w_hh, b_ih, b_hh)]
    arrs = [(ctypes.c_void_p * 2)(*(t.data_ptr() for t in pair)) for pair in keep]
    outs = [[torch.empty_like(t) for t in keep[i]] for i in (0, 1, 2)]
    oarrs = [(ctypes.c_void_p * 2)(*(t.data_ptr() for t in pair)) for pair in outs]
    dx = torch.empty_like(x_) if need_dx else None
    faults = ctypes.c_int(0)
    L.check(lib.dimx_op_lstm_layer_bwd(L.F32, L.ptr(x_), B, T, In, H, arrs[0], arrs[1], arrs[2], arrs[3], L.ptr(dy_), L.ptr(dx),
                                       oarrs[0], oarrs[1], oarrs[2], 1 if safe else 0, ctypes.byref(faults), L.stream_ptr(dev)),
            "dimx_op_lstm_layer_bwd")
    out = (dx, tuple(outs[0]), tuple(outs[1]), tuple(outs[2]))
    return out + (faults.value,) if return_faults else out


def op_layernorm(x, gamma, beta=None, out_bf16=False):
    lib = L.load()
    M, C = x.shape
    y = torch.empty(M, C, dtype=torch.bfloat16 if out_bf16 else torch.float32, device=x.device)
    L.check(lib.dimx_op_layernorm(L.BF16 if out_bf16 else L.F32, L.ptr(x.contiguous()), L.ptr(y), L.ptr(gamma),
                                  L.ptr(beta), M, C, L.stream_ptr(x.device)), "dimx_op_layernorm")
    return y


def op_instnorm(x, lens=None, out_bf16=False):
    lib = L.load()
    B, T, C = x.shape
    y = torch.empty(B, T, C, dtype=torch.bfloat16 if out_bf16 else torch.float32, device=x.device)
    L.check(lib.dimx_op_instnorm(L.BF16 if out_bf16 else L.F32, L.ptr(x.contiguous()), L.ptr(y), L.ptr(lens), B, T,
                                 C, L.stream_ptr(x.device)), "dimx_op_instnorm")
    return y


ATTN_CANARY = -7.0


def _op_attention_strided(q, k, v, scale, causal, lens, kmask, layout, tp, ld_o, prepacked, kmask_ld, return_buffer):
    lib = L.load()
    B, Lq, H, D = q.shape
    Lk = k.shape[1]
    dev, bf, nan = q.device, torch.bfloat16, float("nan")
    ld_o = H * D if ld_o is None else ld_o

    def packed(t, n):
        buf = torch.full((B * n + 8, H * D), nan, dtype=bf, device=dev)
        buf[:B * n] = t.to(bf).reshape(B * n, H * D)
        return buf, (n * H * D, H * D, D)

    q_, q_str = packed(q, Lq)
    if layout == "packed":
        (k_, k_str), (v_, v_str) = packed(k, Lk), packed(v, Lk)
    elif layout == "headmajor":
        tp = Lk if tp is None else tp
        assert tp >= Lk
        k_, v_ = (torch.full((B, H, tp, D), nan, dtype=bf, device=dev) for _ in range(2))
        k_[:, :, :Lk] = k.to(bf).permute(0, 2, 1, 3)
        v_[:, :, :Lk] = v.to(bf).permute(0, 2, 1, 3)
        k_str = v_str = (H * tp * D, D, tp * D)
    else:
        raise ValueError("op_attention: layout %r" % (layout,))
    out = torch.full((B, Lq + 2, ld_o), ATTN_CANARY, dtype=bf, device=dev)
    o_str = ((Lq + 2) * ld_o, ld_o, D)
    km = None
    if kmask is not None:
        kmask_ld = Lk if kmask_ld is None else kmask_ld
        km = torch.ones(B, kmask_ld, dtype=torch.uint8, device=dev)
        km[:, :Lk] = kmask
    arr = lambda s: (ctypes.c_long * 3)(*s)
    L.check(lib.dimx_op_attention_strided(L.ptr(q_), L.ptr(k_), L.ptr(v_), L.ptr(out), B, H, Lq, Lk, D, arr(q_str), arr(k_str),
                                          arr(v_str), arr(o_str), float(scale), 1 if causal else 0, L.ptr(lens), L.ptr(km),
                                          kmask_ld if km is not None else 0, 1 if prepacked else 0, L.stream_ptr(dev)),
            "dimx_op_attention_strided")
    res = out[:, :Lq, :H * D].reshape(B, Lq, H, D)
    return (res, out) if return_buffer else res


def op_attention(q, k, v, scale, causal=False, lens=None, kmask=None, bf16=False, row_v=False, layout=None, tp=None, ld_o=None,
                 prepacked=False, kmask_ld=None, return_buffer=False):
    if layout is not None:
        return _op_attention_strided(q, k, v, scale, causal, lens, kmask, layout, tp, ld_o, prepacked, kmask_ld, return_buffer)
    lib = L.load()
    B, Lq, H, D = q.shape
    Lk = k.shape[1]
    if row_v:
        q_, k_, v_ = (t.to(torch.bfloat16).reshape(B, -1, H * D).contiguous() for t in (q, k, v))
        out = torch.empty(B, Lq, H * D, dtype=torch.bfloat16, device=q.device)
        L.check(lib.dimx_op_attention_rowv(L.ptr(q_), L.ptr(k_), L.ptr(v_), L.ptr(out), B, H, Lq, Lk, D, H * D, H * D, H * D, H * D,
                                           float(scale), 1 if causal else 0, L.ptr(lens), L.ptr(kmask), L.stream_ptr(q.device)),
                "dimx_op_attention_rowv")
        return out.view(B, Lq, H, D)
    dt = torch.bfloat16 if bf16 else torch.float32
    Lp = (Lk + 7) // 8 * 8
    q_ = q.to(dt).reshape(B, Lq, H * D).contiguous()
    k_ = k.to(dt).reshape(B, Lk, H * D).contiguous()
    vt = torch.full((B, H, D, Lp), float("nan"), dtype=dt, device=q.device)
    vt[..., :Lk] = v.to(dt).permute(0, 2, 3, 1)
    out = torch.empty(B, Lq, H * D, dtype=dt, device=q.device)
    L.check(lib.dimx_op_attention(L.BF16 if bf16 else L.F32, L.ptr(q_), L.ptr(k_), L.ptr(vt), L.ptr(out), B, H, Lq,
                                  Lk, D, H * D, H * D, Lp, H * D, float(scale), 1 if causal else 0, L.ptr(lens),
                                  L.ptr(kmask), L.stream_ptr(q.device)), "dimx_op_attention")
    return out.view(B, Lq, H, D)


def op_train_attention(q, k, v, scale, d_o=None, causal=False, kmask=None, kmask2=None, mfma=False, lookahead=None):
    lib = L.load()
# ... 832 lines not shown
```

### dyadic-interaction-modeling_amd/lib.py

```python
import ctypes
import os
from ctypes import (POINTER, c_char_p, c_float, c_int, c_int32, c_int64, c_size_t, c_uint64,
                    c_void_p)

import torch

HERE = os.path.dirname(os.path.abspath(__file__))
LIB_PATH = os.environ.get("DIMX_LIB", os.path.join(HERE, "libdimx_hip.so"))

MODE_PARITY_F32 = 0
MODE_PERF_BF16 = 1
F32, BF16 = 0, 1
ACT_NONE, ACT_LEAKY, ACT_GELU_TANH, ACT_GELU_ERF = 0, 1, 2, 3


class DimxError(RuntimeError):
    pass


class Dims(ctypes.Structure):
    _fields_ = [(n, c_int) for n in (
        "vq_in_dim", "vq_hidden", "vq_layers", "vq_heads", "vq_inter", "vq_n_embed", "vq_zdim",
        "dim_in", "dim", "dim_a", "enc_depth", "dec_depth", "heads", "dim_head", "num_tokens",
        "max_seq_len", "ff_mult", "variant", "spk_in_dim", "spk_hidden", "spk_heads", "spk_inter",
# ... 43 lines not shown
    "dimx_stream_workspace_bytes_prompt": (c_size_t, [c_void_p, c_int, c_int]),
    "dimx_stream_begin_prompted": (c_int, [c_void_p, c_void_p, c_int, c_int, c_void_p, c_void_p, c_int, c_int, c_int, c_int, c_float, c_int,
                                           c_void_p, c_uint64, c_void_p, c_size_t, c_void_p]),
    "dimx_stream_push": (c_int, [c_void_p, c_void_p, c_void_p, c_int, c_void_p, c_int, c_void_p, c_void_p, POINTER(c_int), c_void_p]),
    "dimx_stream_end": (c_int, [c_void_p, c_void_p, c_int, c_void_p, POINTER(c_int), c_void_p]),
    "dimx_stream_abort": (c_int, [c_void_p]),
    "dimx_stream_state": (c_int, [c_void_p, POINTER(c_int), POINTER(c_int), POINTER(c_int)]),
    "dimx_stream_set_events": (c_int, [c_void_p, c_void_p, c_void_p, c_void_p, c_void_p]),
    "dimx_encode_ctx": (c_int, [c_void_p, c_void_p, c_void_p, c_void_p, c_int, c_int, c_int, c_void_p,
                                c_void_p, c_size_t, c_void_p]),
    "dimx_legacy_speaker_features": (c_int, [c_void_p, c_void_p, c_void_p, c_int, c_int, c_void_p, c_void_p,
                                             c_void_p, c_size_t, c_void_p]),
    "dimx_slm_encode": (c_int, [c_void_p, c_void_p, c_void_p, c_void_p, c_void_p, c_void_p, c_int, c_int, c_void_p,
                                c_void_p, c_void_p, c_void_p, c_size_t, c_void_p]),
    "dimx_set_context": (c_int, [c_void_p, c_void_p, c_int, c_int, c_void_p, c_int, c_int, c_int, c_void_p, c_size_t,
                                 c_void_p]),
    "dimx_decode_tf": (c_int, [c_void_p, c_void_p, c_void_p, c_void_p, c_int, c_int, c_void_p, c_void_p,
                               c_void_p, c_void_p, c_size_t, c_void_p]),
    "dimx_decode_tf_win": (c_int, [c_void_p, c_void_p, c_void_p, c_int, c_int, c_int, c_void_p, c_void_p, c_void_p, c_void_p,
                                   c_size_t, c_void_p]),
    "dimx_generate": (c_int, [c_void_p, c_void_p, c_void_p, c_int, c_int, c_int, c_float, c_int, c_void_p, c_uint64,
                              c_void_p, c_void_p, c_void_p, c_size_t, c_void_p]),
    "dimx_workspace_bytes_prompt": (c_size_t, [c_void_p, c_int, c_int, c_int, c_int]),
    "dimx_generate_prompted": (c_int, [c_void_p, c_void_p, c_int, c_void_p, c_int, c_int, c_void_p, c_int, c_int, c_int, c_float,
                                       c_int, c_void_p, c_uint64, c_void_p, c_void_p, c_int, c_void_p, c_size_t, c_void_p]),
    "dimx_generate_beam": (c_int, [c_void_p, c_void_p, c_int, c_void_p, c_int, c_int, c_void_p, c_void_p, c_int, c_int, c_int, c_void_p,
                                   c_void_p, c_void_p, c_void_p, c_void_p, c_size_t, c_int, c_void_p, c_size_t, c_void_p]),
    "dimx_workspace_bytes_guided": (c_size_t, [c_void_p, c_int, c_int]),
    "dimx_generate_guided": (c_int, [c_void_p, c_void_p, c_int, c_void_p, c_int, c_void_p, c_int, c_int, c_float, c_float, c_int, c_void_p,
                                     c_uint64, c_void_p, c_void_p, c_void_p, c_void_p, c_size_t, c_void_p]),
    "dimx_train_num_params": (c_int, [c_void_p]),
    "dimx_train_total": (c_int64, [c_void_p]),
    "dimx_train_param_info": (c_int, [c_void_p, c_int, POINTER(c_char_p), POINTER(c_int64), POINTER(c_int64)]),
    "dimx_train_workspace_bytes": (c_size_t, [c_void_p, c_int, c_int]),
    "dimx_train_forward_backward": (c_int, [c_void_p, c_void_p, c_void_p, c_void_p, c_void_p, c_void_p, c_void_p, c_void_p, c_int,
                                            c_int, c_void_p, c_void_p, c_void_p, c_size_t, c_void_p]),
    "dimx_train_graph_stats": (c_int, [c_void_p, c_void_p]),
    "dimx_set_train_lookahead": (c_int, [c_void_p, c_int, c_int]),
    "dimx_train_lookahead": (c_int, [c_void_p, POINTER(c_int), POINTER(c_int)]),
    "dimx_set_train_cond_keep": (c_int, [c_void_p, c_void_p]),
    "dimx_train_cond_keep": (c_int, [c_void_p, POINTER(c_void_p)]),
    "dimx_train_legacy_workspace_bytes": (c_size_t, [c_void_p, c_int, c_int]),
    "dimx_train_legacy_forward_backward": (c_int, [c_void_p, c_void_p, c_void_p, c_void_p, c_void_p, c_void_p, c_void_p, c_void_p, c_void_p,
                                                   c_void_p, c_int, c_int, c_void_p, c_void_p, c_void_p, c_void_p, c_size_t, c_void_p]),
    "dimx_train_slm_workspace_bytes": (c_size_t, [c_void_p, c_int, c_int]),
    "dimx_train_slm_forward_backward": (c_int, [c_void_p] + [c_void_p] * 14 + [c_int, c_int, c_void_p, c_void_p, c_size_t, c_void_p]),
    "dimx_train_vq_num_params": (c_int, [c_void_p, c_int]),
    "dimx_train_vq_total": (c_int64, [c_void_p, c_int]),
    "dimx_train_vq_param_info": (c_int, [c_void_p, c_int, c_int, POINTER(c_char_p), POINTER(c_int64), POINTER(c_int64)]),
    "dimx_train_vq_workspace_bytes": (c_size_t, [c_void_p, c_int, c_int]),
    "dimx_train_vq_forward_backward": (c_int, [c_void_p, c_int, c_void_p, c_void_p, c_void_p, c_int, c_int, c_float, c_float, c_float,
                                               c_uint64, c_int64, c_void_p, c_void_p, c_void_p, c_void_p, c_size_t, c_void_p]),
    "dimx_train_conv_num_params": (c_int, [c_void_p]),
    "dimx_train_conv_total": (c_int64, [c_void_p]),
    "dimx_train_conv_param_info": (c_int, [c_void_p, c_int, POINTER(c_char_p), POINTER(c_int64), POINTER(c_int64)]),
    "dimx_train_conv_workspace_bytes": (c_size_t, [c_void_p, c_int, c_int]),
    "dimx_train_conv_forward_backward": (c_int, [c_void_p, c_void_p, c_void_p, c_void_p, c_void_p, c_void_p, c_void_p, c_int, c_int, c_int,
                                                 c_int, c_void_p, c_void_p, c_void_p, c_size_t, c_void_p]),
    "dimx_train_spk_num_params": (c_int, [c_void_p]),
    "dimx_train_spk_total": (c_int64, [c_void_p]),
    "dimx_train_spk_param_info": (c_int, [c_void_p, c_int, POINTER(c_char_p), POINTER(c_int64), POINTER(c_int64)]),
    "dimx_train_spk_workspace_bytes": (c_size_t, [c_void_p, c_int, c_int]),
    "dimx_train_spk_forward_backward": (c_int, [c_void_p] + [c_void_p] * 9 + [c_int, c_int, c_void_p, c_void_p, c_void_p, c_void_p, c_void_p,
                                                c_size_t, c_void_p]),
    "dimx_op_lstm_layer_bwd": (c_int, [c_int, c_void_p, c_int, c_int, c_int, c_int, POINTER(c_void_p), POINTER(c_void_p),
                                       POINTER(c_void_p), POINTER(c_void_p), c_void_p, c_void_p, POINTER(c_void_p), POINTER(c_void_p),
                                       POINTER(c_void_p), c_int, POINTER(c_int), c_void_p]),
    "dimx_train_adamw": (c_int, [c_void_p, c_void_p, c_void_p, c_void_p, c_int64, c_float, c_float, c_float, c_float, c_float,
                                 c_int, c_float, c_void_p, c_void_p]),
    "dimx_op_train_attention": (c_int, [c_int, c_void_p, c_void_p, c_void_p, c_void_p, c_void_p, c_void_p, c_int, c_int, c_int,
                                        c_int, c_int, c_float, c_void_p, c_void_p, c_void_p, c_void_p, c_void_p, c_void_p,
                                        c_void_p]),
    "dimx_op_train_attention_win": (c_int, [c_int, c_void_p, c_void_p, c_void_p, c_void_p, c_void_p, c_void_p, c_int, c_int, c_int,
                                            c_int, c_int, c_float, c_int, c_int, c_void_p, c_void_p, c_void_p, c_void_p, c_void_p,
                                            c_void_p, c_void_p]),
    "dimx_op_train_layernorm_bwd": (c_int, [c_void_p, c_void_p, c_void_p, c_void_p, c_int, c_int, c_int, c_void_p, c_void_p, c_void_p,
                                            c_size_t, c_void_p]),
    "dimx_op_train_colsum": (c_int, [c_void_p, c_int, c_int, c_void_p, c_void_p, c_size_t, c_void_p]),
    "dimx_op_train_prep": (c_int, [c_int, c_int, c_void_p, c_int, c_void_p, c_int, c_void_p, c_void_p, c_int, c_int, c_void_p, c_size_t,
                                   c_void_p, c_size_t, c_void_p, c_size_t, POINTER(c_int), c_void_p]),
    "dimx_op_train_cross_entropy": (c_int, [c_void_p, c_void_p, c_int, c_void_p, c_void_p, c_void_p, c_void_p]),
    "dimx_chain_faults": (c_int, [c_void_p]),
    "dimx_qkv0_table_builds": (c_int, [c_void_p]),
    "dimx_kv0_table_generations": (c_int, [c_void_p]),
    "dimx_sample_head_generations": (c_int, [c_void_p]),
    "dimx_lstm_faults": (c_int, [c_void_p]),
    "dimx_mesh_head": (c_int, [c_void_p, c_void_p, c_void_p, c_int, c_int, c_void_p, c_int, c_void_p, c_size_t, c_void_p]),
    "dimx_op_lstm_layer": (c_int, [c_int, c_void_p, c_int, c_int, c_int, c_int, POINTER(c_void_p), POINTER(c_void_p),
                                   POINTER(c_void_p), POINTER(c_void_p), c_void_p, c_int, POINTER(c_int), c_void_p]),
    "dimx_debug_chain_fault": (c_int, [c_void_p, c_int]),
    "dimx_op_gemm_slabs": (c_int, [c_int, c_int, c_int, c_int, c_int]),
    "dimx_op_split_x3": (c_int, [c_void_p, c_void_p, ctypes.c_long, c_void_p]),
    "dimx_op_gemm_x3": (c_int, [c_void_p, c_int, c_void_p, c_void_p, c_int, c_int, c_int, c_int, c_void_p, c_int, c_void_p, c_int, c_int,
                                c_void_p]),
    "dimx_op_gemm": (c_int, [c_int, c_int, c_void_p, c_int, c_void_p, c_int, c_void_p, c_int, c_int, c_int,
                             c_int, c_void_p, c_int, c_void_p, c_int, c_int, c_void_p, c_int, c_void_p]),
    "dimx_op_gemm_headmajor": (c_int, [c_int, c_void_p, c_int, c_void_p, c_int, c_void_p, c_int, c_int, c_int, c_int, c_int,
                                       c_int, c_void_p]),
    "dimx_op_layernorm": (c_int, [c_int, c_void_p, c_void_p, c_void_p, c_void_p, c_int, c_int, c_void_p]),
    "dimx_op_instnorm": (c_int, [c_int, c_void_p, c_void_p, c_void_p, c_int, c_int, c_int, c_void_p]),
    "dimx_op_attention": (c_int, [c_int, c_void_p, c_void_p, c_void_p, c_void_p, c_int, c_int, c_int, c_int,
                                  c_int, c_int, c_int, c_int, c_int, c_float, c_int, c_void_p, c_void_p,
                                  c_void_p]),
    "dimx_op_attention_rowv": (c_int, [c_void_p, c_void_p, c_void_p, c_void_p, c_int, c_int, c_int, c_int, c_int, c_int, c_int,
                                       c_int, c_int, c_float, c_int, c_void_p, c_void_p, c_void_p]),
    "dimx_op_attention_strided": (c_int, [c_void_p, c_void_p, c_void_p, c_void_p, c_int, c_int, c_int, c_int, c_int,
                                          POINTER(ctypes.c_long), POINTER(ctypes.c_long), POINTER(ctypes.c_long), POINTER(ctypes.c_long),
                                          c_float, c_int, c_void_p, c_void_p, c_int, c_int, c_void_p]),
    "dimx_op_decode_attn": (c_int, [c_int, c_void_p, c_void_p, c_void_p, c_void_p, c_int, c_int, c_int, c_int,
                                    c_float, c_void_p, c_int, c_int, c_void_p]),
    "dimx_op_append_attn": (c_int, [c_int, c_void_p, c_int, c_void_p, c_void_p, c_void_p, c_int, c_int, c_int, c_int, c_int, c_float,
                                    c_void_p]),
    "dimx_op_cross_attn_win": (c_int, [c_int, c_void_p, c_int, c_void_p, c_void_p, c_int, c_void_p, c_int, c_int, c_int, c_int, c_int, c_int,
                                       c_int, c_void_p, c_int, c_float, c_void_p]),
    "dimx_op_decode_attn_self": (c_int, [c_int, c_void_p, c_int, c_void_p, c_void_p, c_void_p, c_int, c_int, c_int,
                                         c_void_p, c_float, c_int, c_void_p]),
    "dimx_op_decode_attn_ex": (c_int, [c_int, c_void_p, c_int, c_int, c_int, ctypes.c_long, c_int, c_void_p, c_void_p, c_void_p,
                                       c_int, c_int, c_int, c_int, c_void_p, c_int, c_void_p, c_int, c_int, c_float, c_int,
                                       c_void_p]),
    "dimx_op_decode_attn_win": (c_int, [c_int, c_void_p, c_int, c_int, c_int, ctypes.c_long, c_void_p, c_void_p, c_void_p,
                                        c_int, c_int, c_int, c_int, c_void_p, c_int, c_void_p, c_int, c_int, c_float, c_int,
                                        c_int, c_void_p]),
    "dimx_op_decode_attn_tab": (c_int, [c_int, c_void_p, c_int, c_int, c_int, ctypes.c_long, c_void_p, c_void_p, c_void_p, c_int, c_int,
                                        c_int, c_int, c_void_p, c_float, c_int, c_void_p, c_int, c_int, c_int, c_int, c_void_p, c_int,
                                        c_void_p]),
    "dimx_op_mlp_fused": (c_int, [c_void_p, c_void_p, c_void_p, c_void_p, c_void_p, c_void_p, c_void_p, c_int, c_int, c_int, c_int, c_void_p]),
    "dimx_mlp_fused_packed_bytes": (c_size_t, [c_int, c_int]),
    "dimx_mlp_fused_pack": (c_int, [c_void_p, c_void_p, c_void_p, c_int, c_int, c_void_p, c_size_t]),
    "dimx_op_mlp_fused_packed": (c_int, [c_void_p, c_void_p, c_void_p, c_void_p, c_void_p, c_int, c_int, c_int, c_int, c_void_p]),
    "dimx_op_add_slabs_layernorm": (c_int, [c_int, c_void_p, c_void_p, c_int, ctypes.c_long, c_void_p, c_void_p, c_int,
                                            c_int, c_void_p]),
    "dimx_op_chain": (c_int, [c_void_p, c_int, c_void_p, c_void_p, c_void_p, c_int, c_void_p, c_void_p, c_void_p, c_int,
                              c_void_p, c_int, c_int, c_void_p, c_void_p]),
    "dimx_op_chain_ln": (c_int, [c_void_p, c_int, c_void_p, c_void_p, c_void_p, c_void_p, c_void_p, c_void_p, c_int,
                                 c_void_p, c_int, c_int, c_void_p, c_void_p]),
    "dimx_op_layer_chain": (c_int, [c_void_p, c_int, ctypes.c_long, c_void_p, c_void_p, c_int, c_void_p, c_void_p, c_int, c_int, c_void_p,
                                    c_void_p, c_void_p, c_void_p, c_void_p, c_void_p, c_void_p, c_void_p, c_void_p, c_void_p, c_int,
                                    c_void_p, c_int, c_float, c_void_p, c_void_p, c_void_p]),
    "dimx_op_layer_chain_tab": (c_int, [c_void_p, c_int, ctypes.c_long, c_void_p, c_void_p, c_int, c_void_p, c_void_p, c_int, c_int, c_void_p,
                                        c_void_p, c_void_p, c_void_p, c_void_p, c_void_p, c_void_p, c_void_p, c_void_p, c_void_p, c_int,
                                        c_void_p, c_int, c_float, c_void_p, c_void_p, c_void_p, c_int, c_int, c_int, c_int, c_void_p,
                                        c_int, c_void_p]),
    "dimx_op_layer_chain_head": (c_int, [c_void_p, c_void_p, c_int, c_void_p, c_int, c_void_p, c_int, c_void_p, c_void_p, c_void_p, c_void_p,
                                         c_void_p, c_int, c_void_p, c_void_p, c_int, c_int, c_void_p, c_void_p, c_void_p, c_void_p, c_void_p,
                                         c_void_p, c_void_p, c_void_p, c_void_p, c_void_p, c_int, c_float, c_void_p, c_void_p, c_void_p, c_int,
                                         c_int, c_int, c_int, c_void_p, c_int, c_void_p]),
    "dimx_op_sample_step": (c_int, [c_void_p, c_int, c_int, c_void_p, c_int, c_void_p, c_int, c_void_p, c_void_p, c_int, c_void_p, c_void_p,
                                    c_void_p, c_int, c_void_p, c_int, c_void_p, c_void_p]),
    "dimx_op_gemm_ln": (c_int, [c_int, c_void_p, c_void_p, c_void_p, c_int, c_int, c_int, c_void_p, c_int, c_void_p,
                                c_void_p, c_void_p]),
    "dimx_op_fd_select_ws_bytes": (c_size_t, [c_int, c_int, c_int]),
    "dimx_op_fd_select": (c_int, [c_void_p, ctypes.c_long, ctypes.c_long, c_void_p, ctypes.c_long, ctypes.c_long, ctypes.c_long, c_void_p,
                                  c_int, c_int, c_int, c_int, c_int, c_int, c_void_p, c_void_p, c_void_p, c_void_p, c_void_p, c_size_t,
                                  c_void_p]),
    "dimx_op_mesh_metrics_ws_bytes": (c_size_t, [c_int, c_int, c_int, c_int]),
    "dimx_op_mesh_metrics": (c_int, [c_void_p, ctypes.c_long, ctypes.c_long, c_void_p, ctypes.c_long, ctypes.c_long, c_void_p, ctypes.c_long,
                                     POINTER(c_int32), c_int, c_int, c_int, c_void_p, c_int, c_void_p, c_int, c_void_p, c_void_p, c_void_p,
                                     c_void_p, c_size_t, c_void_p]),
    "dimx_op_listener_metrics_ws_bytes": (c_size_t, [c_int, c_int, c_int]),
    "dimx_op_listener_metrics": (c_int, [c_void_p, ctypes.c_long, ctypes.c_long, c_void_p, ctypes.c_long, ctypes.c_long, c_void_p, ctypes.c_long,
                                         ctypes.c_long, c_void_p, c_int, c_int, c_int, c_int, POINTER(c_int32), c_int, c_void_p, c_void_p,
                                         c_void_p, c_size_t, c_void_p]),
    "dimx_op_kmeans_fit_ws_bytes": (c_size_t, [c_int, c_int, c_int]),
    "dimx_op_kmeans_fit": (c_int, [c_void_p, ctypes.c_long, c_int, c_int, c_int, c_int, c_int, c_int, c_void_p, c_int, ctypes.c_double,
                                   c_int, c_void_p, c_void_p, c_void_p, c_void_p, c_void_p, c_size_t, c_void_p]),
    "dimx_op_sid_assign": (c_int, [c_void_p, ctypes.c_long, c_int, c_int, c_int, c_int, c_void_p, c_int, c_void_p, c_void_p, c_void_p,
                                   c_void_p]),
    "dimx_op_seq_logprob": (c_int, [c_void_p, ctypes.c_long, ctypes.c_long, c_void_p, ctypes.c_long, c_void_p, c_void_p, c_int, c_int,
                                    c_int, c_void_p, c_void_p, c_void_p, c_void_p]),
    "dimx_op_score_select": (c_int, [c_void_p, c_void_p, ctypes.c_long, ctypes.c_long, ctypes.c_long, c_void_p, c_void_p, ctypes.c_long,
                                     c_int, c_int, c_int, c_int, c_int, c_void_p, c_void_p, c_void_p, c_void_p, c_void_p]),
    "dimx_op_consensus_select_ws_bytes": (c_size_t, [c_int, c_int, c_int, c_int]),
    "dimx_op_consensus_select": (c_int, [c_void_p, ctypes.c_long, ctypes.c_long, ctypes.c_long, c_void_p, c_int, c_int, c_int, c_int, c_int,
                                         c_int, c_int, c_void_p, c_void_p, c_void_p, c_void_p, c_void_p, c_void_p, ctypes.c_long, c_int,
                                         c_void_p, c_void_p, c_size_t, c_void_p]),
    "dimx_op_pool_desc": (c_int, [c_void_p, ctypes.c_long, ctypes.c_long, c_void_p, c_int, c_int, c_int, c_int, c_void_p, c_void_p,
                                  c_void_p]),
    "dimx_op_nn_search_ws_bytes": (c_size_t, [c_int, c_int, c_int, c_int]),
    "dimx_op_nn_search": (c_int, [c_void_p, ctypes.c_long, c_void_p, c_void_p, ctypes.c_long, c_void_p, c_int, c_int, c_int, c_int,
                                  c_void_p, c_void_p, c_void_p, c_void_p, c_void_p, c_size_t, c_void_p]),
    "dimx_op_nn_gather": (c_int, [c_void_p, c_void_p, ctypes.c_long, ctypes.c_long, c_void_p, c_void_p, c_int, c_int, c_int, c_int,
                                  c_int, c_int, c_void_p, c_void_p, c_void_p]),
    "dimx_op_beam_step": (c_int, [c_void_p, c_void_p, c_void_p, c_void_p, c_int, c_int, c_void_p, c_void_p, c_void_p, c_void_p]),
    "dimx_op_beam_reorder": (c_int, [c_void_p, c_int, c_void_p, c_int, c_int, c_int, c_int, c_int, c_void_p]),
    "dimx_op_sample": (c_int, [c_void_p, c_int, c_int, c_float, c_void_p, c_uint64, c_uint64, c_void_p,
                               c_void_p]),
    "dimx_op_sample_guided": (c_int, [c_void_p, c_void_p, c_int, c_int, ctypes.c_long, c_float, c_int, c_int, c_float, c_float, c_float,
                                      c_void_p, c_uint64, c_uint64, c_void_p, c_void_p, c_void_p]),
    "dimx_op_sample_filtered": (c_int, [c_void_p, c_int, c_int, c_int, c_float, c_float, c_float, c_void_p, c_uint64, c_uint64,
                                        c_void_p, c_void_p, c_void_p]),
}

_lib = None


def load(build_if_missing=True):
    global _lib
    if _lib is not None:
        return _lib
    in_tree = "DIMX_LIB" not in os.environ
    if not os.path.exists(LIB_PATH):
        if not build_if_missing or not in_tree:
            raise DimxError("libdimx_hip.so not found at %s (run python __graft_entry__.py build)" % LIB_PATH)
        from . import build as _build
        _build.build()
    elif in_tree:
        from . import build as _build
        if _build.stale():
            if build_if_missing and _build.have_hipcc():
                _build.build()
            elif not os.environ.get("DIMX_ALLOW_STALE_LIB"):
                raise DimxError("libdimx_hip.so at %s was not built from the sources next to it and %s; run "
# ... 61 lines not shown
```

### include/dimx.h

```cpp
#ifndef DIMX_H
#define DIMX_H

#include <stddef.h>
#include <stdint.h>

#ifdef __cplusplus
extern "C" {
#endif

typedef struct dimx_ctx* dimx_handle;

typedef enum {
    DIMX_OK = 0,
    DIMX_ERR_ARG = -1,
    DIMX_ERR_HIP = -2,
    DIMX_ERR_WEIGHT = -3,
    DIMX_ERR_STATE = -4,
    DIMX_ERR_WORKSPACE = -5
} dimx_status;

#define DIMX_MODE_PARITY_F32 0
#define DIMX_MODE_PERF_BF16 1

#define DIMX_F32 0
// ... 40 lines not shown
int dimx_vq_decode(dimx_handle h, int which, const int32_t* idx, int B, int L, int batch_row_offset,
                   int rows_per_clip, float* out, void* ws, size_t ws_bytes, void* stream);

int dimx_vq_decode_latent(dimx_handle h, int which, const float* z, int B, int L, int batch_row_offset,
                          float* out, void* ws, size_t ws_bytes, void* stream);

int dimx_encode_speaker(dimx_handle h, const float* v_speaker, const uint8_t* mask, int B, int T,
                        float* x_s_out, void* ws, size_t ws_bytes, void* stream);

int dimx_set_shard(dimx_handle h, int row_offset, int rows_total);

int dimx_encode_ctx(dimx_handle h, const float* v_speaker, const float* v_audio, const uint8_t* mask,
                    int B, int T, int for_generate, float* x_s_out, void* ws, size_t ws_bytes,
                    void* stream);

int dimx_slm_encode(dimx_handle h, const float* v_speaker, const float* v_listener, const uint8_t* mask,
                    const uint8_t* mask_speaker, const uint8_t* mask_listener, int B, int T, float* x_s,
                    float* x_l, float* x_joint, void* ws, size_t ws_bytes, void* stream);

int dimx_set_context(dimx_handle h, const float* x, int ldx_rows, int which_patch, const float* v_audio, int B,
                     int T, int for_generate, void* ws, size_t ws_bytes, void* stream);

int dimx_legacy_speaker_features(dimx_handle h, const float* v_speaker, const uint8_t* mask, int B, int T,
                                 float* x_speaker_out, int32_t* idx_out, void* ws, size_t ws_bytes,
                                 void* stream);

int dimx_decode_tf(dimx_handle h, const int32_t* z_l, const uint8_t* ctx_mask, const uint8_t* kv_mask,
                   int B, int T, float* logits, float* row_loss, int32_t* argmax_tok, void* ws,
                   size_t ws_bytes, void* stream);

int dimx_decode_tf_win(dimx_handle h, const int32_t* z_l, const uint8_t* ctx_mask, int B, int T, int lookahead, float* logits,
                       float* row_loss, int32_t* argmax_tok, void* ws, size_t ws_bytes, void* stream);

int dimx_generate(dimx_handle h, const int32_t* start, const uint8_t* ctx_mask, int B, int T, int n_samples,
                  float temperature, int top_k, const float* exp_noise, uint64_t seed, int32_t* tokens,
                  float* logits_out, void* ws, size_t ws_bytes, void* stream);

size_t dimx_workspace_bytes_prompt(dimx_handle h, int B, int T, int n_samples, int P0);
int dimx_generate_prompted(dimx_handle h, const int32_t* prompt, int ld_prompt, const int32_t* prompt_len, int Pmax, int P0,
                           const uint8_t* ctx_mask, int B, int T, int n_samples, float temperature, int top_k,
                           const float* exp_noise, uint64_t seed, int32_t* tokens, float* logits_out, int flags, void* ws,
                           size_t ws_bytes, void* stream);

#define DIMX_BEAM_STATE_BYTES(B, W) ((size_t)16 * (size_t)(B) * (size_t)(W))
int dimx_generate_beam(dimx_handle h, const int32_t* prompt, int ld_prompt, const int32_t* prompt_len, int Pmax, int P0,
                       const uint8_t* ctx_mask, const int32_t* lens, int B, int T, int beam_width, int32_t* tokens, double* scores,
                       int32_t* backptr, float* logits_out, void* beam_state, size_t beam_state_bytes, int flags, void* ws, size_t ws_bytes,
                       void* stream);

size_t dimx_workspace_bytes_guided(dimx_handle h, int B, int T);
int dimx_generate_guided(dimx_handle h, const int32_t* prompt, int ld_prompt, const int32_t* prompt_len, int Pmax, const uint8_t* ctx_mask,
                         int B, int T, float scale, float temperature, int top_k, const float* exp_noise, uint64_t seed, int32_t* tokens,
                         float* logits_out, float* branch_logits_out, void* ws, size_t ws_bytes, void* stream);

int dimx_chain_faults(dimx_handle h);

typedef enum {
    DIMX_FILTER_TOP_K = 0,
    DIMX_FILTER_TOP_P = 1,
    DIMX_FILTER_MIN_P = 2,
    DIMX_FILTER_TOP_A = 3
} dimx_filter_kind;
int dimx_set_sampler_filter(dimx_handle h, int kind, float a, float b);

int dimx_set_cross_lookahead(dimx_handle h, int on, int lookahead);
int dimx_cross_lookahead(dimx_handle h, int* on, int* lookahead);
size_t dimx_cross_kv8_bytes(dimx_handle h, int B, int T);
int dimx_set_cross_kv8(dimx_handle h, void* buf, size_t bytes);
int dimx_cross_kv8(dimx_handle h, void** buf, size_t* bytes);
size_t dimx_stream_workspace_bytes(dimx_handle h, int B, int Tmax);
int dimx_stream_begin(dimx_handle h, const int32_t* start, int B, int Tmax, int lookahead, float temperature, int top_k, const float* noise,
                      uint64_t seed, void* ws, size_t ws_bytes, void* stream);
size_t dimx_stream_workspace_bytes_prompt(dimx_handle h, int B, int Tmax);
int dimx_stream_begin_prompted(dimx_handle h, const int32_t* prompt, int ld_prompt, int P, const float* v_speaker, const float* v_audio, int F,
                               int B, int Tmax, int lookahead, float temperature, int top_k, const float* noise, uint64_t seed, void* ws,
                               size_t ws_bytes, void* stream);
int dimx_stream_push(dimx_handle h, const float* v_speaker, const float* v_audio, int c, int32_t* tokens_out, int ld_tok, float* logits_out,
                     float* x_s_out, int* n_new, void* stream);
int dimx_stream_end(dimx_handle h, int32_t* tokens_out, int ld_tok, float* logits_out, int* n_new, void* stream);
int dimx_stream_abort(dimx_handle h);
int dimx_stream_state(dimx_handle h, int* frames, int* steps, int* open);
int dimx_stream_set_events(dimx_handle h, void* ev_start, void* ev_encoded, void* ev_appended, void* ev_stepped);
int dimx_qkv0_table_builds(dimx_handle h);
int dimx_kv0_table_generations(dimx_handle h);
int dimx_sample_head_generations(dimx_handle h);
int dimx_debug_chain_fault(dimx_handle h, int n_calls);

int dimx_mesh_head(dimx_handle h, const float* motion, const float* templ, int B, int L, float* mesh_out, int flags, void* ws,
                   size_t ws_bytes, void* stream);
int dimx_lstm_faults(dimx_handle h);

int dimx_train_num_params(dimx_handle h);
int64_t dimx_train_total(dimx_handle h);
int dimx_train_param_info(dimx_handle h, int i, const char** name, int64_t* offset, int64_t* numel);
size_t dimx_train_workspace_bytes(dimx_handle h, int B, int T);
int dimx_train_forward_backward(dimx_handle h, const float* params, float* grads, const float* v_speaker, const float* v_audio,
                                const uint8_t* mask, const int32_t* z_l, const uint8_t* kv_mask, int B, int T, float* loss_out,
                                float* logits_out, void* ws, size_t ws_bytes, void* stream);
int dimx_train_graph_stats(dimx_handle h, int64_t* out3);
int dimx_set_train_lookahead(dimx_handle h, int on, int lookahead);
int dimx_train_lookahead(dimx_handle h, int* on, int* lookahead);
int dimx_set_train_cond_keep(dimx_handle h, const uint8_t* keep_dev);
int dimx_train_cond_keep(dimx_handle h, const uint8_t** keep_dev);
size_t dimx_train_legacy_workspace_bytes(dimx_handle h, int B, int T);
int dimx_train_legacy_forward_backward(dimx_handle h, const float* params, float* grads, const float* x_speaker, const int32_t* z_l,
                                       const float* v_listener, const uint8_t* mask, const int32_t* listener_ids, const float* codebook,
                                       const float* pe, int B, int T, float* loss_out, float* pred_out, float* logits_out, void* ws,
                                       size_t ws_bytes, void* stream);
size_t dimx_train_slm_workspace_bytes(dimx_handle h, int B, int T);
int dimx_train_slm_forward_backward(dimx_handle h, const float* params, float* grads, const float* v_speaker, const float* v_listener,
                                    const float* v_audio, const uint8_t* mask, const uint8_t* mask_speaker, const uint8_t* mask_listener,
                                    const int32_t* z_s, const int32_t* z_l, const float* codebook_s, const float* codebook_l,
                                    const float* pe_s, const float* pe_l, int B, int T, float* loss_out, void* ws, size_t ws_bytes,
                                    void* stream);
int dimx_train_vq_num_params(dimx_handle h, int which);
int64_t dimx_train_vq_total(dimx_handle h, int which);
int dimx_train_vq_param_info(dimx_handle h, int which, int i, const char** name, int64_t* offset, int64_t* numel);
size_t dimx_train_vq_workspace_bytes(dimx_handle h, int B, int T);
int dimx_train_vq_forward_backward(dimx_handle h, int which, const float* params, float* grads, const float* x, int B, int T, float beta,
                                   float quant_loss_weight, float dropout_p, uint64_t dropout_seed, int64_t step, float* loss_out,
                                   float* pred_out, int32_t* idx_out, void* ws, size_t ws_bytes, void* stream);
int dimx_train_conv_num_params(dimx_handle h);
int64_t dimx_train_conv_total(dimx_handle h);
int dimx_train_conv_param_info(dimx_handle h, int i, const char** name, int64_t* offset, int64_t* numel);
size_t dimx_train_conv_workspace_bytes(dimx_handle h, int B, int T);
int dimx_train_conv_forward_backward(dimx_handle h, const float* params, float* grads, const float* motion, const float* templ,
                                     const float* target, const float* vert_w, int n_mouth, int B, int T, int flags, float* loss_out,
                                     float* mesh_out, void* ws, size_t ws_bytes, void* stream);
int dimx_train_spk_num_params(dimx_handle h);
int64_t dimx_train_spk_total(dimx_handle h);
int dimx_train_spk_param_info(dimx_handle h, int i, const char** name, int64_t* offset, int64_t* numel);
size_t dimx_train_spk_workspace_bytes(dimx_handle h, int B, int T);
int dimx_train_spk_forward_backward(dimx_handle h, const float* params, float* grads, const float* v_emoca, const float* v_audio,
                                    const uint8_t* mask, const int32_t* z, const int32_t* speaker_ids, const float* codebook_s,
                                    const float* pe_s, int B, int T, float* loss_out, float* logits_out, int32_t* idx_out, float* pred_out,
                                    void* ws, size_t ws_bytes, void* stream);
int dimx_op_lstm_layer_bwd(int dtype, const float* x, int B, int T, int In, int H, const float* const* w_ih, const float* const* w_hh,
                           const float* const* b_ih, const float* const* b_hh, const float* dy, float* dx, float* const* dw_ih,
                           float* const* dw_hh, float* const* db, int flags, int* faults_out, void* stream);
int dimx_train_adamw(float* params, const float* grads, float* exp_avg, float* exp_avg_sq, int64_t n, float lr, float beta1,
                     float beta2, float eps, float weight_decay, int step, float max_norm, float* scratch, void* stream);
int dimx_op_train_attention(int mfma, const float* q, const float* k, const float* v, const float* d_o, const uint8_t* kmask,
                            const uint8_t* kmask2, int B, int H, int Lq, int Lk, int causal, float scale, float* o, float* lse,
                            float* delta, float* dq, float* dk, float* dv, void* stream);
int dimx_op_train_attention_win(int mfma, const float* q, const float* k, const float* v, const float* d_o, const uint8_t* kmask,
                                const uint8_t* kmask2, int B, int H, int Lq, int Lk, int causal, float scale, int win, int lookahead,
                                float* o, float* lse, float* delta, float* dq, float* dk, float* dv, void* stream);
int dimx_op_train_layernorm_bwd(const float* x, const float* gamma, const float* dy, float* dx, int accumulate, int M, int C, float* dgamma,
                                float* dbeta, float* scratch, size_t scratch_floats, void* stream);
int dimx_op_train_colsum(const float* dy, int M, int C, float* out, float* scratch, size_t scratch_floats, void* stream);
int dimx_op_train_prep(int dtype, int mode, const float* src, int lds, const float* src2, int lds2, const float* gamma, const float* beta,
                       int rows, int cols, void* o, size_t o_elems, void* t, size_t t_elems, float* colpart, size_t colpart_floats,
                       int* dims3, void* stream);
int dimx_op_train_cross_entropy(const float* logits, const int32_t* targets, int R, float* row_loss, float* dlogits, float* loss_out2,
                                void* stream);


int dimx_op_gemm(int in_dtype, int out_dtype, const void* A, int lda, const void* W, int ldw, void* C,
                 int ldc, int M, int N, int K, const float* bias, int act, const float* residual,
                 int ldr, int conv_T, const int32_t* conv_lens, int flags, void* stream);
int dimx_op_split_x3(const float* w, void* planes, long n, void* stream);
int dimx_op_gemm_x3(const float* A, int lda, const void* planes, float* C, int ldc, int M, int N, int K, const float* bias, int act,
                    const float* residual, int ldr, int flags, void* stream);
int dimx_op_gemm_slabs(int in_dtype, int M, int N, int K, int flags);
int dimx_op_gemm_headmajor(int dtype, const void* A, int lda, const void* W, int ldw, void* out, int M, int N, int K,
                           int rowT, int Tp, int nlayers, void* stream);
int dimx_op_lstm_layer(int dtype, const float* x, int B, int T, int In, int H, const float* const* w_ih, const float* const* w_hh,
                       const float* const* b_ih, const float* const* b_hh, float* y, int flags, int* faults_out, void* stream);
int dimx_op_layernorm(int out_dtype, const float* x, void* y, const float* gamma, const float* beta,
                      int M, int C, void* stream);
int dimx_op_instnorm(int out_dtype, const float* x, void* y, const int32_t* lens, int B, int T, int C,
                     void* stream);
int dimx_op_attention(int dtype, const void* q, const void* k, const void* vt, void* out, int B, int H,
                      int Lq, int Lk, int D, int ldq, int ldk, int ld_vt, int ldo, float scale,
                      int causal, const int32_t* lens, const uint8_t* kmask, void* stream);
int dimx_op_attention_rowv(const void* q, const void* k, const void* v, void* out, int B, int H, int Lq, int Lk, int D, int ldq,
                           int ldk, int ldv, int ldo, float scale, int causal, const int32_t* lens, const uint8_t* kmask,
                           void* stream);
int dimx_op_attention_strided(const void* q, const void* k, const void* v, void* out, int B, int H, int Lq, int Lk, int D,
                              const long* q_str, const long* k_str, const long* v_str, const long* o_str, float scale, int causal,
                              const int32_t* lens, const uint8_t* kmask, int kmask_ld, int prepacked, void* stream);
int dimx_op_decode_attn(int dtype, const void* q, const void* kcache, const void* vcache, void* out, int B, int H,
                        int Tmax, int n_keys, float scale, const uint8_t* kmask, int nsplit, int q_is_f32,
                        void* stream);
int dimx_op_decode_attn_self(int dtype, const void* qkv, int ld, void* kcache, void* vcache, void* out, int B, int H,
                             int Tmax, const int32_t* step_dev, float scale, int q_is_f32, void* stream);
int dimx_op_decode_attn_ex(int dtype, const void* q, int q_ld, int q_is_f32, int nslab, long slab_stride, int self_attn, void* kcache,
                           void* vcache, void* out, int o_ld, int B, int H, int Tmax, const int32_t* step_dev, int n_keys,
                           const uint8_t* kmask, int kmask_ld, int rows_per_clip, float scale, int nsplit, void* stream);
int dimx_op_decode_attn_tab(int dtype, const void* q, int q_ld, int q_is_f32, int nslab, long slab_stride, void* kcache, void* vcache,
                            void* out, int o_ld, int B, int H, int Tmax, const int32_t* step_dev, float scale, int nsplit, const void* tab,
                            int tab_ld, int tab_koff, int tab_voff, int tab_rows, const int32_t* hist, int hist_ld, void* stream);
int dimx_op_decode_attn_win(int dtype, const void* q, int q_ld, int q_is_f32, int nslab, long slab_stride, void* kcache, void* vcache,
                            void* out, int o_ld, int B, int H, int Tmax, const int32_t* step_dev, int n_keys, const uint8_t* kmask,
                            int kmask_ld, int rows_per_clip, float scale, int nsplit, int lookahead, void* stream);
int dimx_op_kv8_quantize(int dtype, const void* cache, int B, int H, int Tp, int T, uint8_t* codes, float* scales, void* stream);
int dimx_op_decode_attn_kv8(int out_dtype, const void* q, int q_ld, int q_is_f32, int nslab, long slab_stride, const uint8_t* kcodes,
                            const float* kscale, const uint8_t* vcodes, const float* vscale, void* out, int o_ld, int B, int H, int Tmax,
                            const int32_t* step_dev, int n_keys, const uint8_t* kmask, int kmask_ld, int rows_per_clip, float scale, int nsplit,
                            int lookahead, int win, void* stream);
int dimx_op_append_attn(int dtype, const float* qkv, int ld, void* kcache, void* vcache, void* out, int B, int H, int Tmax, int n0, int c,
                        float scale, void* stream);
int dimx_op_cross_attn_win(int dtype, const float* q, int ld, const void* kcache, const void* vcache, int Tp, void* out, int o_ld, int B, int H,
                           int Lq, int t0, int n_keys, int lookahead, const uint8_t* kmask, int kmask_ld, float scale, void* stream);
int dimx_op_mlp_fused(float* x, const float* w1_host, const float* b1_host, const float* w2_host, const float* b2, const float* ln_g,
                      const float* ln_b, int M, int C, int F, int act, void* stream);
size_t dimx_mlp_fused_packed_bytes(int C, int F);
int dimx_mlp_fused_pack(const float* w1_host, const float* b1_host, const float* w2_host, int C, int F, void* out_host, size_t out_bytes);
int dimx_op_mlp_fused_packed(float* x, const void* packed, const float* b2, const float* ln_g, const float* ln_b, int M, int C, int F,
                             int act, void* stream);
int dimx_op_add_slabs_layernorm(int out_dtype, float* x, const float* slabs, int nslab, long slab_stride, void* y,
                                const float* gamma, int M, int C, void* stream);
int dimx_op_chain(const void* A1, int K1, const void* W1, float* x, const float* slabs, int nslab, const float* gamma,
                  void* y, const void* W2, int N2, float* out2, int B, int C, void* scratch, void* stream);
int dimx_op_chain_ln(const void* A1, int K1, const void* W1, float* x, void* y, float* stats, const void* W2s,
                     const float* colsum2, int N2, float* out2, int B, int C, void* scratch, void* stream);
int dimx_op_gemm_ln(int out_dtype, const void* A, const void* Ws, void* C, int M, int N, int K, const float* bias, int act,
                    const float* stats, const float* colsum, void* stream);
int dimx_op_layer_chain(const float* qkv, int nslab, long slab_stride, void* sk, void* sv, int T, const void* ck, const void* cv,
                        int Tp, int n_keys, const uint8_t* kmask, const void* w_so, const void* w_cq, const float* colsum_cq,
                        const void* w_co, float* x, void* y, void* o, float* qc, float* stats, int B, const int32_t* step,
                        int call_index, float scale, void* scratch, void* prof, void* stream);
int dimx_op_layer_chain_tab(const float* qkv, int nslab, long slab_stride, void* sk, void* sv, int T, const void* ck, const void* cv,
                            int Tp, int n_keys, const uint8_t* kmask, const void* w_so, const void* w_cq, const float* colsum_cq,
                            const void* w_co, float* x, void* y, void* o, float* qc, float* stats, int B, const int32_t* step,
                            int call_index, float scale, void* scratch, void* prof, const void* tab, int tab_ld, int tab_koff,
                            int tab_voff, int tab_rows, const int32_t* hist, int hist_ld, void* stream);
int dimx_op_layer_chain_head(const float* qkv0, const float* logits, int top_k, const float* exp_noise, int rows_total, int32_t* tokens,
                             int tok_ld, float* logits_out, const float* emb_table, int32_t* params, void* sk, void* sv, int T, const void* ck,
                             const void* cv, int Tp, int n_keys, const uint8_t* kmask, const void* w_so, const void* w_cq,
                             const float* colsum_cq, const void* w_co, float* x, void* y, void* o, float* qc, float* stats, int B, float scale,
                             void* scratch, void* prof, const void* tab, int tab_ld, int tab_koff, int tab_voff, int tab_rows, int32_t* hist,
                             int hist_ld, void* stream);
int dimx_op_sample_step(const float* logits, int R, int top_k, const float* exp_noise, int rows_total, int32_t* tokens, int tok_ld,
                        float* logits_out, const float* emb_table, int C, float* x_next, const float* qkv0, float* qkv0_out, int qkv0_N,
                        int32_t* hist, int hist_ld, int32_t* params, void* stream);
size_t dimx_op_fd_select_ws_bytes(int B, int S, int F);
int dimx_op_fd_select(const float* y_true, long yt_clip_stride, long yt_frame_stride, const float* y_pred, long yp_clip_stride,
                      long yp_sample_stride, long yp_frame_stride, const int32_t* lens, int B, int S, int L, int W, int c0, int F,
                      double* fd, int32_t* win, uint8_t* ok, float* best, void* workspace, size_t workspace_bytes, void* stream);
size_t dimx_op_mesh_metrics_ws_bytes(int B, int L, int n_mouth, int n_upper);
int dimx_op_mesh_metrics(const float* y_true, long yt_clip_stride, long yt_frame_stride, const float* y_pred, long yp_clip_stride,
                         long yp_frame_stride, const float* templ, long templ_clip_stride, const int32_t* lens, int B, int L, int n_vert,
                         const int32_t* mouth, int n_mouth, const int32_t* upper, int n_upper, double* clip_out, double* frame_max,
                         int32_t* status, void* workspace, size_t workspace_bytes, void* stream);
#define DIMX_LM_ROW 133
size_t dimx_op_listener_metrics_ws_bytes(int B, int n_win, int F);
int dimx_op_listener_metrics(const float* y_true, long yt_clip_stride, long yt_frame_stride, const float* y_pred, long yp_clip_stride,
                             long yp_frame_stride, const float* x, long x_clip_stride, long x_frame_stride, const int32_t* lens, int B,
                             int L, int Wy, int Wx, const int32_t* windows, int n_win, double* fd, double* moments, void* workspace,
                             size_t workspace_bytes, void* stream);
size_t dimx_op_kmeans_fit_ws_bytes(int N, int K, int F);
int dimx_op_kmeans_fit(const float* frames, long frame_stride, int N, int W, int c0, int F, int K, int first_index, const double* U,
                       int trials, double tol, int max_iter, double* centers, int32_t* n_iter, int32_t* status, int32_t* labels,
                       void* workspace, size_t workspace_bytes, void* stream);
int dimx_op_sid_assign(const float* frames, long frame_stride, int M, int W, int c0, int F, const double* centers, int K, int64_t* hist,
                       double* sid, int32_t* labels, void* stream);
int dimx_op_seq_logprob(const float* logits, long row_stride, long step_stride, const int32_t* tokens, long tok_row_stride,
                        const int32_t* first, const int32_t* last, int rows_per_clip, int R, int n, double* tok_logprob, double* score,
                        int32_t* count, void* stream);
int dimx_op_score_select(const double* score, const float* y_pred, long yp_clip_stride, long yp_sample_stride, long yp_frame_stride,
                         const int32_t* lens, const int32_t* tokens, long tok_row_stride, int B, int S, int L, int W, int n,
                         int32_t* win, uint8_t* ok, float* best, int32_t* best_tokens, void* stream);
size_t dimx_op_consensus_select_ws_bytes(int B, int S, int F, int kind);
int dimx_op_consensus_select(const float* y_pred, long yp_clip_stride, long yp_sample_stride, long yp_frame_stride,
                             const int32_t* lens, int B, int S, int L, int W, int c0, int F, int kind ,
                             double* dist , double* risk , int32_t* win, uint8_t* ok,
                             float* best , const int32_t* tokens, long tok_row_stride, int n_tok,
                             int32_t* best_tokens , void* workspace, size_t workspace_bytes, void* stream);
int dimx_op_pool_desc(const float* x, long clip_stride, long frame_stride, const int32_t* lens, int N, int T, int D,
                      int kind , double* desc, double* norm, void* stream);
size_t dimx_op_nn_search_ws_bytes(int Q, int N, int D, int K);
int dimx_op_nn_search(const double* q_desc, long q_row_stride, const double* q_norm, const double* x_desc, long x_row_stride,
                      const double* x_norm, int Q, int N, int D, int K, int32_t* idx, double* sim, int32_t* found,
                      double* sim_out , void* workspace, size_t workspace_bytes, void* stream);
int dimx_op_nn_gather(const int32_t* idx, const float* lib_seq, long clip_stride, long frame_stride, const int32_t* lib_lens,
                      const int32_t* q_lens, int Q, int K, int N, int Lmax, int L, int W, float* out, int32_t* out_len, void* stream);
int dimx_op_beam_step(const float* logits, const double* cum, const int32_t* mode, const int32_t* forced_tok, int B, int W,
                      int32_t* parent, int32_t* token, double* cum_out, void* stream);
int dimx_op_beam_reorder(void* cache, int dtype, const int32_t* parent, int R, int W, int H, int T, int c, void* stream);
int dimx_op_sample(const float* logits, int R, int top_k, float temperature, const float* exp_noise,
                   uint64_t seed, uint64_t step, int32_t* tokens, void* stream);
int dimx_op_sample_filtered(const float* logits, int R, int kind, int top_k, float a, float b, float temperature,
                            const float* exp_noise, uint64_t seed, uint64_t step, int32_t* tokens, uint8_t* keep_out,
                            void* stream);
int dimx_op_sample_guided(const float* cond, const float* uncond, int R, int nslab, long slab_stride, float scale, int kind, int top_k,
                          float a, float b, float temperature, const float* exp_noise, uint64_t seed, uint64_t step, int32_t* tokens,
                          float* guided_out, void* stream);

#ifdef __cplusplus
}
#endif
#endif
// ... 1 lines not shown
```

Measured before the change: 1741 clips/s.

## Fuse pre-attention LayerNorm with QKV projection in a single MFMA kernel

Adds a dedicated kernel that keeps each row's LayerNorm result in registers as bf16 MFMA operands and multiplies it against prepacked QKV weights streamed through LDS with a three-slot pipeline, writing separate Q, K and V bf16 outputs. It replaces a LayerNorm launch plus a separate GEMM in the self-attention QKV path, removing the normalized-activation round trip through global memory. The fused path is enabled by default for bf16 encoder layers with C=384. It covers only that width, and it adds prepacked weight memory and hand-written inline-asm wait counts that must stay correct.

```diff
diff --git a/dyadic-interaction-modeling_amd/build.py b/dyadic-interaction-modeling_amd/build.py
--- a/dyadic-interaction-modeling_amd/build.py
+++ b/dyadic-interaction-modeling_amd/build.py
@@ -7,13 +7,13 @@
 CSRC = os.path.join(HERE, "csrc")
 OBJ = os.path.join(CSRC, "_obj")
 LIB = os.path.join(HERE, "libdimx_hip.so")
-SOURCES = ["gemm.hip", "gemm_x3.hip", "gemm256.hip", "norm.hip", "attention.hip", "attention_tr.hip", "mlp_fused.hip", "decode_attn.hip", "vq.hip", "elementwise.hip", "kv_prefill.hip", "chain.hip", "model.hip", "generate.hip", "ops.hip", "stream_attn.hip", "win_attn.hip", "stream.hip",
+SOURCES = ["gemm.hip", "gemm_x3.hip", "gemm256.hip", "norm.hip", "attention.hip", "attention_tr.hip", "mlp_fused.hip", "ln_qkv.hip", "decode_attn.hip", "vq.hip", "elementwise.hip", "kv_prefill.hip", "chain.hip", "model.hip", "generate.hip", "ops.hip", "stream_attn.hip", "win_attn.hip", "stream.hip",
            "train_kernels.hip", "train_attn.hip", "train_vq.hip", "train.hip", "lstm.hip", "train_lstm.hip", "train_spk.hip", "fd_select.hip", "mesh_metrics.hip",
            "listener_metrics.hip", "kmeans_sid.hip", "seq_score.hip", "beam.hip", "consensus.hip", "retrieval.hip", "decode_attn_kv8.hip"]
 HEADERS = ["common.hpp", "model.hpp", "stages.hpp", "train.hpp", "decode_attn_body.hpp", "sample_pick.hpp", "online_softmax_body.hpp", "frechet.hpp", "pick_gather.hpp", os.path.join("..", "..", "include", "dimx.h")]
 FLAGS = ["--offload-arch=gfx950", "-O3", "-std=c++17", "-fPIC", "-Wall", "-Wno-unused-function",
          "-Wno-unused-variable", "-ffp-contract=on"]
-SRC_FLAGS = {"attention_tr.hip": ["-fno-slp-vectorize"]}
+SRC_FLAGS = {"attention_tr.hip": ["-fno-slp-vectorize"], "ln_qkv.hip": ["-fno-slp-vectorize"]}
 
 
 def _hipcc():
diff --git a/dyadic-interaction-modeling_amd/csrc/common.hpp b/dyadic-interaction-modeling_amd/csrc/common.hpp
--- a/dyadic-interaction-modeling_amd/csrc/common.hpp
+++ b/dyadic-interaction-modeling_amd/csrc/common.hpp
@@ -299,6 +299,10 @@
 int mlp_fused_pack(const float* w1, const float* b1, const float* w2, int C, int F, uint16_t* out);
 int launch_mlp_fused(float* x, const void* packed, const float* b2, const float* ln_g, const float* ln_b, int M, int C, int F, int act,
                      hipStream_t s);
+size_t ln_qkv_packed_bytes(int C, int N);
+int ln_qkv_pack(const float* w, int C, int N, uint16_t* out);
+int launch_ln_qkv(const float* x, const void* packed, const float* bias, const float* ln_g, const float* ln_b, void* q, void* k, void* v,
+                  int M, int C, int N, hipStream_t s);
 
 struct DecodeAttnArgs {
     int dtype;
diff --git a/dyadic-interaction-modeling_amd/csrc/generate.hip b/dyadic-interaction-modeling_amd/csrc/generate.hip
--- a/dyadic-interaction-modeling_amd/csrc/generate.hip
+++ b/dyadic-interaction-modeling_amd/csrc/generate.hip
@@ -1113,6 +1113,7 @@
 
 int dimx_chain_faults(dimx_handle h) { return h ? h->chain_faults : 0; }
 int dimx_qkv0_table_builds(dimx_handle h) { return h ? h->qkv0_builds : 0; }
+int dimx_ln_qkv_launches(dimx_handle h) { return h ? h->ln_qkv_launches : 0; }
 int dimx_kv0_table_generations(dimx_handle h) { return h ? h->kv0_generations : 0; }
 int dimx_sample_head_generations(dimx_handle h) { return h ? h->sample_head_generations : 0; }
 
diff --git a/dyadic-interaction-modeling_amd/csrc/ln_qkv.hip b/dyadic-interaction-modeling_amd/csrc/ln_qkv.hip
--- /dev/null
+++ b/dyadic-interaction-modeling_amd/csrc/ln_qkv.hip
@@ -0,0 +1,276 @@
+#include "common.hpp"
+
+namespace dimx {
+namespace {
+
+typedef unsigned u32x4_t __attribute__((ext_vector_type(4)));
+typedef unsigned u32x2_t __attribute__((ext_vector_type(2)));
+typedef float f32x8_t __attribute__((ext_vector_type(8)));
+typedef __attribute__((address_space(3))) void lds_void_t;
+typedef const __attribute__((address_space(1))) void glb_void_t;
+typedef const __attribute__((address_space(4))) float cfloat_t;
+
+constexpr int kC = 384;
+constexpr int kKS = kC / 16;
+constexpr int kChunkBytes = kKS * 1024;
+constexpr int kSlots = 3;
+constexpr int kScratch = 2048;
+constexpr int kLdsBytes = kSlots * kChunkBytes + 4 * kScratch;
+
+struct LnQkvArgs {
+    const float* x;
+    const void* wp;
+    const float* bias;
+    const float* ln_g;
+    const float* ln_b;
+    bf16* out[3];
+    int M, nchunk, seg_chunks;
+};
+
+template <bool BETA, bool BIAS> __global__ __launch_bounds__(256, 2) void ln_qkv_kernel(const LnQkvArgs a) {
+    extern __shared__ __attribute__((aligned(1024))) unsigned char smem[];
+    const int tid = threadIdx.x, wave = __builtin_amdgcn_readfirstlane(tid >> 6), lane = tid & 63, hf = lane >> 5, l31 = lane & 31;
+    const int row0 = blockIdx.x * 128 + wave * 32;
+    const int rowc = row0 + l31 < a.M ? row0 + l31 : a.M - 1;
+    const bool full = row0 + 32 <= a.M;
+    const unsigned lds0 = (unsigned)(size_t)(lds_void_t*)smem;
+    const int nch = a.nchunk;
+
+    const unsigned char* const wlane = (const unsigned char*)a.wp + lane * 16;
+    auto issue_chunk = [&](int chunk, int slot) {
+        const int cw = chunk < nch ? chunk : chunk - nch;
+#pragma unroll
+        for (int j = 0; j < 6; ++j) {
+            const int p = wave + 4 * j;
+            __builtin_amdgcn_global_load_lds((glb_void_t*)(wlane + (size_t)cw * kChunkBytes + (size_t)p * 1024),
+                                             (lds_void_t*)(smem + slot * kChunkBytes + p * 1024), 16, 0, 0);
+        }
+    };
+    issue_chunk(0, 0);
+    issue_chunk(1, 1);
+    const unsigned gb0 = lds0 + kSlots * kChunkBytes;
+#pragma unroll
+    for (int j = 0; j < 3; ++j) {
+        const int p = wave + 4 * j;
+        if (p < (BETA ? 12 : 6)) {
+            const float* src = (p < 6 ? a.ln_g + 64 * p : a.ln_b + 64 * (p - 6)) + lane;
+            __builtin_amdgcn_global_load_lds((glb_void_t*)src, (lds_void_t*)(smem + kSlots * kChunkBytes + p * 256), 4, 0, 0);
+        }
+    }
+
+    bf16x8_t xb[kKS];
+    {
+        const float* xr = a.x + (size_t)rowc * kC + 8 * hf;
+        f32x4_t v[kKS][2];
+#pragma unroll
+        for (int s = 0; s < kKS; ++s) {
+            v[s][0] = *(const f32x4_t*)(xr + 16 * s);
+            v[s][1] = *(const f32x4_t*)(xr + 16 * s + 4);
+        }
+#define LNQ_X(s, jj) v[s][(jj) >> 1][2 * ((jj)&1)]
+#define LNQ_Y(s, jj) v[s][(jj) >> 1][2 * ((jj)&1) + 1]
+        float quad[8];
+#pragma unroll
+        for (int s0 = 0; s0 < 8; ++s0) {
+            float p[4];
+#pragma unroll
+            for (int jj = 0; jj < 4; ++jj) {
+                float s = 0.f;
+#pragma unroll
+                for (int i = 0; i < 3; ++i) s += LNQ_X(s0 + 8 * i, jj) + LNQ_Y(s0 + 8 * i, jj);
+                p[jj] = s;
+            }
+            quad[s0] = (p[0] + p[1]) + (p[2] + p[3]);
+        }
+        auto finish = [&](float (&qd)[8]) {
+#pragma unroll
+            for (int s0 = 0; s0 < 8; ++s0) qd[s0] += xor_lane_f32<32>(qd[s0]);
+            const float r0 = qd[0] + qd[1], r1 = qd[2] + qd[3], r2 = qd[4] + qd[5], r3 = qd[6] + qd[7];
+            return (r0 + r1) + (r2 + r3);
+        };
+        const float mean = finish(quad) * (1.0f / kC);
+#pragma unroll
+        for (int s0 = 0; s0 < 8; ++s0) {
+            float p[4];
+#pragma unroll
+            for (int jj = 0; jj < 4; ++jj) {
+                float q = 0.f;
+#pragma unroll
+                for (int i = 0; i < 3; ++i) {
+                    const float da = LNQ_X(s0 + 8 * i, jj) - mean, db = LNQ_Y(s0 + 8 * i, jj) - mean;
+                    q += da * da + db * db;
+                }
+                p[jj] = q;
+            }
+            quad[s0] = (p[0] + p[1]) + (p[2] + p[3]);
+        }
+#undef LNQ_X
+#undef LNQ_Y
+        const float rstd = rsqrtf(finish(quad) * (1.0f / kC) + 1e-5f);
+        float mean_n = mean;
+        asm volatile("" : "+v"(mean_n));
+        asm volatile("s_waitcnt vmcnt(0)" ::: "memory");
+        __builtin_amdgcn_s_barrier();
+        const unsigned grd = gb0 + 32 * hf;
+        u32x4_t gb[2][4];
+        auto read_gb = [&](int s, u32x4_t (&d)[4]) {
+            asm volatile("ds_read_b128 %0, %1 offset:%2" : "=v"(d[0]) : "v"(grd), "i"(64 * s));
+            asm volatile("ds_read_b128 %0, %1 offset:%2" : "=v"(d[1]) : "v"(grd), "i"(64 * s + 16));
+            if (BETA) {
+                asm volatile("ds_read_b128 %0, %1 offset:%2" : "=v"(d[2]) : "v"(grd), "i"(kC * 4 + 64 * s));
+                asm volatile("ds_read_b128 %0, %1 offset:%2" : "=v"(d[3]) : "v"(grd), "i"(kC * 4 + 64 * s + 16));
+            }
+        };
+        read_gb(0, gb[0]);
+#pragma unroll
+        for (int s = 0; s < kKS; ++s) {
+            if (s + 1 < kKS) {
+                read_gb(s + 1, gb[(s + 1) & 1]);
+                if (BETA) asm volatile("s_waitcnt lgkmcnt(4)" ::: "memory");
+                else asm volatile("s_waitcnt lgkmcnt(2)" ::: "memory");
+            } else {
+                asm volatile("s_waitcnt lgkmcnt(0)" ::: "memory");
+            }
+            __builtin_amdgcn_sched_barrier(0);
+            const f32x4_t g0 = __builtin_bit_cast(f32x4_t, gb[s & 1][0]), g1 = __builtin_bit_cast(f32x4_t, gb[s & 1][1]);
+            f32x4_t b0 = {0.f, 0.f, 0.f, 0.f}, b1 = {0.f, 0.f, 0.f, 0.f};
+            if (BETA) {
+                b0 = __builtin_bit_cast(f32x4_t, gb[s & 1][2]);
+                b1 = __builtin_bit_cast(f32x4_t, gb[s & 1][3]);
+            }
+            const f32x4_t v0 = v[s][0], v1 = v[s][1];
+            uint32_t w[4];
+#pragma unroll
+            for (int j = 0; j < 2; ++j) {
+                const float o0 = (v0[2 * j] - mean_n) * rstd * g0[2 * j] + b0[2 * j];
+                const float o1 = (v0[2 * j + 1] - mean_n) * rstd * g0[2 * j + 1] + b0[2 * j + 1];
+                const float o2 = (v1[2 * j] - mean_n) * rstd * g1[2 * j] + b1[2 * j];
+                const float o3 = (v1[2 * j + 1] - mean_n) * rstd * g1[2 * j + 1] + b1[2 * j + 1];
+                w[j] = pack_bf16x2(o0, o1);
+                w[2 + j] = pack_bf16x2(o2, o3);
+            }
+            u32x4_t u = {w[0], w[1], w[2], w[3]};
+            asm volatile("" : "+v"(u));
+            xb[s] = __builtin_bit_cast(bf16x8_t, u);
+        }
+        __builtin_amdgcn_sched_barrier(0);
+    }
+
+    const unsigned rd = lds0 + lane * 16;
+    const unsigned sbase = lds0 + kSlots * kChunkBytes + wave * kScratch;
+    const unsigned swr = sbase + (unsigned)(l31 * 64 + hf * 8), swz = (unsigned)((l31 >> 2) & 3);
+    const int srow = lane >> 2, sc16 = lane & 3;
+    const unsigned srd = sbase + (unsigned)(srow * 64 + ((sc16 ^ ((srow >> 2) & 3)) << 4));
+    const int m0 = row0 + srow, m1 = m0 + 16;
+    int slot = 0, slot2 = 2, seg = 0, segc = 0;
+    for (int c = 0; c < nch; ++c) {
+        if (full && c >= 2) asm volatile("s_waitcnt vmcnt(10)" ::: "memory");
+        else asm volatile("s_waitcnt vmcnt(6)" ::: "memory");
+        __builtin_amdgcn_s_barrier();
+        issue_chunk(c + 2, slot2);
+
+        f32x16_t acc;
+#pragma unroll
+        for (int r = 0; r < 16; ++r) acc[r] = 0.f;
+        const unsigned base = rd + slot * kChunkBytes;
+        u32x4_t fr[2][6];
+#pragma unroll
+        for (int q = 0; q < 6; ++q) asm volatile("ds_read_b128 %0, %1 offset:%2" : "=v"(fr[0][q]) : "v"(base), "i"(q * 1024));
+#pragma unroll
+        for (int g = 0; g < 4; ++g) {
+            if (g + 1 < 4) {
+#pragma unroll
+                for (int q = 0; q < 6; ++q)
+                    asm volatile("ds_read_b128 %0, %1 offset:%2" : "=v"(fr[(g + 1) & 1][q]) : "v"(base), "i"(((g + 1) * 6 + q) * 1024));
+                asm volatile("s_waitcnt lgkmcnt(6)" ::: "memory");
+            } else {
+                asm volatile("s_waitcnt lgkmcnt(0)" ::: "memory");
+            }
+            __builtin_amdgcn_sched_barrier(0);
+#pragma unroll
+            for (int q = 0; q < 6; ++q)
+                acc = __builtin_amdgcn_mfma_f32_32x32x16_bf16(__builtin_bit_cast(bf16x8_t, fr[g & 1][q]), xb[g * 6 + q], acc, 0, 0, 0);
+        }
+
+#pragma unroll
+        for (int q = 0; q < 4; ++q) {
+            float v0 = acc[4 * q], v1 = acc[4 * q + 1], v2 = acc[4 * q + 2], v3 = acc[4 * q + 3];
+            if (BIAS) {
+                const f32x8_t bv = *(const __attribute__((address_space(4))) f32x8_t*)(cfloat_t*)(a.bias + 32 * c + 8 * q);
+                v0 += hf ? bv[4] : bv[0];
+                v1 += hf ? bv[5] : bv[1];
+                v2 += hf ? bv[6] : bv[2];
+                v3 += hf ? bv[7] : bv[3];
+            }
+            u32x2_t pk;
+            pk[0] = pack_bf16x2(v0, v1);
+            pk[1] = pack_bf16x2(v2, v3);
+            asm volatile("ds_write_b64 %0, %1" ::"v"(swr + (((unsigned)q ^ swz) << 4)), "v"(pk) : "memory");
+        }
+        asm volatile("s_waitcnt lgkmcnt(0)" ::: "memory");
+        u32x4_t raw0, raw1;
+        asm volatile("ds_read_b128 %0, %1" : "=v"(raw0) : "v"(srd) : "memory");
+        asm volatile("ds_read_b128 %0, %1 offset:1024" : "=v"(raw1) : "v"(srd) : "memory");
+        asm volatile("s_waitcnt lgkmcnt(0)" ::: "memory");
+        __builtin_amdgcn_sched_barrier(0);
+        bf16* const op = a.out[seg] + 32 * segc + 8 * sc16;
+        const size_t ldo = (size_t)a.seg_chunks * 32;
+        if (full) {
+            *(u32x4_t*)(op + (size_t)m0 * ldo) = raw0;
+            *(u32x4_t*)(op + (size_t)m1 * ldo) = raw1;
+        } else {
+            if (m0 < a.M) *(u32x4_t*)(op + (size_t)m0 * ldo) = raw0;
+            if (m1 < a.M) *(u32x4_t*)(op + (size_t)m1 * ldo) = raw1;
+        }
+        slot = slot == 2 ? 0 : slot + 1;
+        slot2 = slot2 == 2 ? 0 : slot2 + 1;
+        if (++segc == a.seg_chunks) {
+            segc = 0;
+            ++seg;
+        }
+    }
+    asm volatile("s_waitcnt vmcnt(0)" ::: "memory");
+}
+
+}
+
+size_t ln_qkv_packed_bytes(int C, int N) { return (C == kC && N > 0 && N % 96 == 0) ? (size_t)(N / 32) * kChunkBytes : 0; }
+
+int ln_qkv_pack(const float* w, int C, int N, uint16_t* out) {
+    DIMX_REQUIRE(C == kC && N > 0 && N % 32 == 0, DIMX_ERR_ARG, "ln_qkv_pack: C = %d N = %d not supported", C, N);
+    for (int c = 0; c < N / 32; ++c)
+        for (int s = 0; s < kKS; ++s)
+            for (int l = 0; l < 64; ++l)
+                for (int j = 0; j < 8; ++j)
+                    out[((size_t)c * kKS + s) * 512 + l * 8 + j] = host_f32_to_bf16(w[(size_t)(32 * c + (l & 31)) * C + 16 * s + 8 * (l >> 5) + j]);
+    return DIMX_OK;
+}
+
+int launch_ln_qkv(const float* x, const void* packed, const float* bias, const float* ln_g, const float* ln_b, void* q, void* k, void* v,
+                  int M, int C, int N, hipStream_t s) {
+    DIMX_REQUIRE(x && packed && ln_g && q && k && v && M > 0, DIMX_ERR_ARG, "ln_qkv: null argument");
+    DIMX_REQUIRE(ln_qkv_packed_bytes(C, N) > 0, DIMX_ERR_ARG, "ln_qkv: C = %d N = %d not supported", C, N);
+    DIMX_REQUIRE(((uintptr_t)x % 16) == 0 && ((uintptr_t)packed % 16) == 0 && ((uintptr_t)ln_g % 16) == 0 && (!ln_b || ((uintptr_t)ln_b % 16) == 0) &&
+                     (!bias || ((uintptr_t)bias % 32) == 0) && ((uintptr_t)q % 16) == 0 && ((uintptr_t)k % 16) == 0 && ((uintptr_t)v % 16) == 0,
+                 DIMX_ERR_ARG, "ln_qkv: operands must be 16-byte aligned (bias: 32)");
+    LnQkvArgs a;
+    a.x = x; a.wp = packed; a.bias = bias; a.ln_g = ln_g; a.ln_b = ln_b;
+    a.out[0] = (bf16*)q; a.out[1] = (bf16*)k; a.out[2] = (bf16*)v;
+    a.M = M; a.nchunk = N / 32; a.seg_chunks = N / 96;
+    const dim3 grid((M + 127) / 128);
+#define LNQ_LAUNCH(A, B)                                                                                                                \
+    do {                                                                                                                                \
+        DIMX_HIP(hipFuncSetAttribute((const void*)ln_qkv_kernel<A, B>, hipFuncAttributeMaxDynamicSharedMemorySize, kLdsBytes));        \
+        hipLaunchKernelGGL((ln_qkv_kernel<A, B>), grid, dim3(256), kLdsBytes, s, a);                                                    \
+    } while (0)
+    if (ln_b) {
+        if (bias) LNQ_LAUNCH(true, true); else LNQ_LAUNCH(true, false);
+    } else {
+        if (bias) LNQ_LAUNCH(false, true); else LNQ_LAUNCH(false, false);
+    }
+#undef LNQ_LAUNCH
+    DIMX_HIP(hipGetLastError());
+    return DIMX_OK;
+}
+
+}
diff --git a/dyadic-interaction-modeling_amd/csrc/model.hip b/dyadic-interaction-modeling_amd/csrc/model.hip
--- a/dyadic-interaction-modeling_amd/csrc/model.hip
+++ b/dyadic-interaction-modeling_amd/csrc/model.hip
@@ -338,6 +338,33 @@
     return DIMX_OK;
 }
 
+static int pack_ln_qkv(dimx_ctx* c, const std::vector<std::string>& parts, const void** out) {
+    *out = nullptr;
+    if (c->at != DIMX_BF16) return DIMX_OK;
+    int N = 0, C = -1;
+    for (const auto& n : parts) {
+        auto it = c->host.find(n);
+        DIMX_REQUIRE(it != c->host.end(), DIMX_ERR_WEIGHT, "missing weight %s", n.c_str());
+        const auto& sh = it->second.shape;
+        if (sh.size() != 2 || (C >= 0 && C != (int)sh[1]) || sh[0] % 32 != 0) return DIMX_OK;
+        C = (int)sh[1];
+        N += (int)sh[0];
+    }
+    const size_t bytes = ln_qkv_packed_bytes(C, N);
+    if (bytes == 0) return DIMX_OK;
+    std::vector<uint16_t> img(bytes / 2);
+    size_t row = 0;
+    for (const auto& n : parts) {
+        const HostTensor& t = c->host[n];
+        DIMX_TRY(ln_qkv_pack(t.data.data(), C, (int)t.shape[0], img.data() + row * C));
+        row += (size_t)t.shape[0];
+    }
+    void* p;
+    DIMX_TRY(dev_upload(c, img.data(), bytes, &p));
+    *out = p;
+    return DIMX_OK;
+}
+
 static int pack_vq(dimx_ctx* c, int which) {
     VQNet& v = c->vq[which];
     const VQGeom& vg = c->vqg[which];
@@ -361,6 +388,7 @@
             DIMX_TRY(upload_f32(c, a + "norm.weight", &blk[i].ln1_g));
             DIMX_TRY(upload_f32(c, a + "norm.bias", &blk[i].ln1_b));
             DIMX_TRY(pack_linear(c, {a + "fn.to_qkv.weight"}, "", false, &blk[i].qkv));
+            DIMX_TRY(pack_ln_qkv(c, {a + "fn.to_qkv.weight"}, &blk[i].ln_qkv));
             DIMX_TRY(pack_linear(c, {a + "fn.to_out.weight"}, a + "fn.to_out.bias", false, &blk[i].out));
             DIMX_TRY(upload_f32(c, m + "norm.weight", &blk[i].ln2_g));
             DIMX_TRY(upload_f32(c, m + "norm.bias", &blk[i].ln2_b));
@@ -394,10 +422,12 @@
 
 static int pack_xattn(dimx_ctx* c, const std::string& p, bool cross, XAttn* a) {
     DIMX_TRY(upload_f32(c, p + "0.0.weight", &a->ln_g));
+    a->ln_qkv = nullptr;
     if (cross) {
         DIMX_TRY(pack_linear(c, {p + "1.to_q.weight"}, "", false, &a->qkv));
     } else {
         DIMX_TRY(pack_linear(c, {p + "1.to_q.weight", p + "1.to_k.weight", p + "1.to_v.weight"}, "", false, &a->qkv));
+        DIMX_TRY(pack_ln_qkv(c, {p + "1.to_q.weight", p + "1.to_k.weight", p + "1.to_v.weight"}, &a->ln_qkv));
     }
     DIMX_TRY(pack_linear(c, {p + "1.to_out.weight"}, "", false, &a->out));
     return DIMX_OK;
@@ -672,9 +702,17 @@
     return residual_linear(c, b.f, f1.N, f2, M, b.h, C, st);
 }
 
+constexpr int kLnQkvMinRows = 16384;
+
 int self_attn_qkv(const dimx_ctx* c, const BlockBufs& b, const float* ln_g, const float* ln_b, const Linear& qkv, int B,
-                         int T, int C, int heads, int D, AttnArgs& a, hipStream_t st) {
+                         int T, int C, int heads, int D, AttnArgs& a, hipStream_t st, const void* ln_qkv) {
     const bool rowv = qkv_row_v(c->at, D);
+    if (ln_qkv && c->use_ln_qkv && c->at == DIMX_BF16 && rowv && C == 384 && qkv.N == 3 * heads * D && B * T >= kLnQkvMinRows) {
+        DIMX_TRY(launch_ln_qkv(b.h, ln_qkv, qkv.bias, ln_g, ln_b, b.q, b.k, b.vt, B * T, C, qkv.N, st));
+        ++c->ln_qkv_launches;
+        set_attn_packed(a, c->at, b.q, b.k, b.vt, b.o, B, heads, T, T, D, tpad(T), rowv);
+        return DIMX_OK;
+    }
     DIMX_TRY(launch_layernorm(c->at, b.h, b.y, ln_g, ln_b, B * T, C, st));
     GemmArgs g;
     gemm_lin(c, b.y, C, qkv, B * T, g);
@@ -736,7 +774,7 @@
     for (int l = 0; l < vg.layers; ++l) {
         const VQBlock& b = blk[l];
         AttnArgs a;
-        DIMX_TRY(self_attn_qkv(c, s, b.ln1_g, b.ln1_b, b.qkv, B, T, Hd, heads, D, a, st));
+        DIMX_TRY(self_attn_qkv(c, s, b.ln1_g, b.ln1_b, b.qkv, B, T, Hd, heads, D, a, st, b.ln_qkv));
         a.scale = scale; a.lens = lens;
         DIMX_TRY(attn_out(c, s, a, b.out, Hd, st));
         DIMX_TRY(ff_sublayer(c, s, b.ln2_g, b.ln2_b, b.l1, b.l2, b.mlp, ACT_GELU_TANH, M, Hd, st));
@@ -869,6 +907,7 @@
     c->use_qkv0_table = getenv("DIMX_NO_QKV0_TABLE") ? 0 : 1;
     c->use_kv0_table = getenv("DIMX_NO_KV0_TABLE") ? 0 : 1;
     c->use_sample_head = getenv("DIMX_NO_SAMPLE_HEAD") ? 0 : 1;
+    c->use_ln_qkv = getenv("DIMX_NO_LN_QKV") ? 0 : 1;
     if (getenv("DIMX_LAYER_PROF")) {
         void* p = nullptr;
         if (hipMalloc(&p, (size_t)8 * 256 * 16 * 8) == hipSuccess) {
@@ -1227,7 +1266,7 @@
     DIMX_TRY(launch_gemm(g, st));
     for (int l = 0; l < eg.depth; ++l) {
         AttnArgs a;
-        DIMX_TRY(self_attn_qkv(c, s, e.attn[l].ln_g, nullptr, e.attn[l].qkv, B, T, dim, heads, D, a, st));
+        DIMX_TRY(self_attn_qkv(c, s, e.attn[l].ln_g, nullptr, e.attn[l].qkv, B, T, dim, heads, D, a, st, e.attn[l].ln_qkv));
         a.scale = 1.0f / sqrtf((float)D); a.causal = eg.causal; a.kmask = mask; a.kmask_ld = T;
         DIMX_TRY(attn_out(c, s, a, e.attn[l].out, dim, st));
         DIMX_TRY(ff_sublayer(c, s, e.ff[l].ln_g, nullptr, e.ff[l].f1, e.ff[l].f2, e.ff[l].mlp, ACT_GELU_ERF, M, dim, st));
diff --git a/dyadic-interaction-modeling_amd/csrc/model.hpp b/dyadic-interaction-modeling_amd/csrc/model.hpp
--- a/dyadic-interaction-modeling_amd/csrc/model.hpp
+++ b/dyadic-interaction-modeling_amd/csrc/model.hpp
@@ -18,6 +18,7 @@
     const float *ln1_g, *ln1_b, *ln2_g, *ln2_b;
     Linear qkv, out, l1, l2;
     const void* mlp = nullptr;
+    const void* ln_qkv = nullptr;
 };
 
 struct VQNet {
@@ -35,6 +36,7 @@
 struct XAttn {
     const float* ln_g;
     Linear qkv;
+    const void* ln_qkv = nullptr;
     Linear kv;
     Linear out;
     Linear q_ln;
@@ -220,6 +222,8 @@
     void* kv0_image = nullptr;
     int kv0_generations = 0;
     int use_sample_head = 1;
+    int use_ln_qkv = 1;
+    mutable int ln_qkv_launches = 0;
     int sample_head_generations = 0;
     int shard_row_off = 0, shard_rows_total = 0;
     int filter_kind = 0;
diff --git a/dyadic-interaction-modeling_amd/csrc/ops.hip b/dyadic-interaction-modeling_amd/csrc/ops.hip
--- a/dyadic-interaction-modeling_amd/csrc/ops.hip
+++ b/dyadic-interaction-modeling_amd/csrc/ops.hip
@@ -468,6 +468,37 @@
     int rc = DIMX_OK;
     if (hipMemcpy(p, img.data(), bytes, hipMemcpyHostToDevice) != hipSuccess) rc = DIMX_ERR_HIP;
     if (rc == DIMX_OK) rc = launch_mlp_fused(x, p, b2, ln_g, ln_b, M, C, F, act, (hipStream_t)stream);
+    if (hipStreamSynchronize((hipStream_t)stream) != hipSuccess && rc == DIMX_OK) rc = DIMX_ERR_HIP;
+    (void)hipFree(p);
+    return rc;
+}
+
+size_t dimx_ln_qkv_packed_bytes(int C, int N) { return ln_qkv_packed_bytes(C, N); }
+
+int dimx_ln_qkv_pack(const float* w_host, int C, int N, void* out_host, size_t out_bytes) {
+    DIMX_REQUIRE(w_host && out_host, DIMX_ERR_ARG, "ln_qkv_pack: null argument");
+    DIMX_REQUIRE(ln_qkv_packed_bytes(C, N) > 0 && out_bytes >= ln_qkv_packed_bytes(C, N), DIMX_ERR_ARG,
+                 "ln_qkv_pack: C = %d N = %d unsupported or the output buffer is too small", C, N);
+    return ln_qkv_pack(w_host, C, N, (uint16_t*)out_host);
+}
+
+int dimx_op_ln_qkv_packed(const float* x, const void* packed, const float* bias, const float* ln_g, const float* ln_b, void* q, void* k,
+                          void* v, int M, int C, int N, void* stream) {
+    return launch_ln_qkv(x, packed, bias, ln_g, ln_b, q, k, v, M, C, N, (hipStream_t)stream);
+}
+
+int dimx_op_ln_qkv(const float* x, const float* w_host, const float* bias, const float* ln_g, const float* ln_b, void* q, void* k, void* v,
+                   int M, int C, int N, void* stream) {
+    DIMX_REQUIRE(x && w_host && ln_g && q && k && v && M > 0, DIMX_ERR_ARG, "op_ln_qkv: null argument");
+    const size_t bytes = ln_qkv_packed_bytes(C, N);
+    DIMX_REQUIRE(bytes > 0, DIMX_ERR_ARG, "op_ln_qkv: C = %d N = %d not supported", C, N);
+    std::vector<uint16_t> img(bytes / 2);
+    DIMX_TRY(ln_qkv_pack(w_host, C, N, img.data()));
+    void* p = nullptr;
+    DIMX_HIP(hipMalloc(&p, bytes));
+    int rc = DIMX_OK;
+    if (hipMemcpy(p, img.data(), bytes, hipMemcpyHostToDevice) != hipSuccess) rc = DIMX_ERR_HIP;
+    if (rc == DIMX_OK) rc = launch_ln_qkv(x, p, bias, ln_g, ln_b, q, k, v, M, C, N, (hipStream_t)stream);
     if (hipStreamSynchronize((hipStream_t)stream) != hipSuccess && rc == DIMX_OK) rc = DIMX_ERR_HIP;
     (void)hipFree(p);
     return rc;
diff --git a/dyadic-interaction-modeling_amd/csrc/stages.hpp b/dyadic-interaction-modeling_amd/csrc/stages.hpp
--- a/dyadic-interaction-modeling_amd/csrc/stages.hpp
+++ b/dyadic-interaction-modeling_amd/csrc/stages.hpp
@@ -23,7 +23,7 @@
 int ff_sublayer(const dimx_ctx* c, const BlockBufs& b, const float* ln_g, const float* ln_b, const Linear& f1, const Linear& f2,
                 const void* mlp, int act, int M, int C, hipStream_t st);
 int self_attn_qkv(const dimx_ctx* c, const BlockBufs& b, const float* ln_g, const float* ln_b, const Linear& qkv, int B, int T, int C,
-                  int heads, int D, AttnArgs& a, hipStream_t st);
+                  int heads, int D, AttnArgs& a, hipStream_t st, const void* ln_qkv = nullptr);
 int attn_out(const dimx_ctx* c, const BlockBufs& b, AttnArgs& a, const Linear& out, int C, hipStream_t st);
 int cross_attn_sublayer(const dimx_ctx* c, const BlockBufs& b, const XAttn& x, AttnArgs& a, const uint8_t* ctx_mask, int C, hipStream_t st,
                         const float* v_rows = nullptr);
diff --git a/dyadic-interaction-modeling_amd/engine.py b/dyadic-interaction-modeling_amd/engine.py
--- a/dyadic-interaction-modeling_amd/engine.py
+++ b/dyadic-interaction-modeling_amd/engine.py
@@ -442,6 +442,9 @@
     def qkv0_table_builds(self):
         return int(self.lib.dimx_qkv0_table_builds(self.h))
 
+    def ln_qkv_launches(self):
+        return int(self.lib.dimx_ln_qkv_launches(self.h))
+
     def kv0_table_generations(self):
         return int(self.lib.dimx_kv0_table_generations(self.h))
 
@@ -719,6 +722,18 @@
     L.check(lib.dimx_op_layernorm(L.BF16 if out_bf16 else L.F32, L.ptr(x.contiguous()), L.ptr(y), L.ptr(gamma),
                                   L.ptr(beta), M, C, L.stream_ptr(x.device)), "dimx_op_layernorm")
     return y
+
+
+def op_ln_qkv(x, w, gamma, beta=None, bias=None, tail_rows=0):
+    lib = L.load()
+    dev = x.device
+    M, C = x.shape
+    N = w.shape[0]
+    w_ = w.detach().to("cpu", torch.float32).contiguous()
+    outs = [torch.full((M + tail_rows, N // 3), float("nan"), dtype=torch.bfloat16, device=dev) for _ in range(3)]
+    L.check(lib.dimx_op_ln_qkv(L.ptr(x.contiguous()), ctypes.c_void_p(w_.data_ptr()), L.ptr(bias), L.ptr(gamma), L.ptr(beta),
+                               L.ptr(outs[0]), L.ptr(outs[1]), L.ptr(outs[2]), M, C, N, L.stream_ptr(dev)), "dimx_op_ln_qkv")
+    return tuple(outs)
 
 
 def op_instnorm(x, lens=None, out_bf16=False):
diff --git a/dyadic-interaction-modeling_amd/lib.py b/dyadic-interaction-modeling_amd/lib.py
--- a/dyadic-interaction-modeling_amd/lib.py
+++ b/dyadic-interaction-modeling_amd/lib.py
@@ -149,6 +149,7 @@
     "dimx_op_train_cross_entropy": (c_int, [c_void_p, c_void_p, c_int, c_void_p, c_void_p, c_void_p, c_void_p]),
     "dimx_chain_faults": (c_int, [c_void_p]),
     "dimx_qkv0_table_builds": (c_int, [c_void_p]),
+    "dimx_ln_qkv_launches": (c_int, [c_void_p]),
     "dimx_kv0_table_generations": (c_int, [c_void_p]),
     "dimx_sample_head_generations": (c_int, [c_void_p]),
     "dimx_lstm_faults": (c_int, [c_void_p]),
@@ -195,6 +196,10 @@
     "dimx_mlp_fused_packed_bytes": (c_size_t, [c_int, c_int]),
     "dimx_mlp_fused_pack": (c_int, [c_void_p, c_void_p, c_void_p, c_int, c_int, c_void_p, c_size_t]),
     "dimx_op_mlp_fused_packed": (c_int, [c_void_p, c_void_p, c_void_p, c_void_p, c_void_p, c_int, c_int, c_int, c_int, c_void_p]),
+    "dimx_op_ln_qkv": (c_int, [c_void_p, c_void_p, c_void_p, c_void_p, c_void_p, c_void_p, c_void_p, c_void_p, c_int, c_int, c_int, c_void_p]),
+    "dimx_ln_qkv_packed_bytes": (c_size_t, [c_int, c_int]),
+    "dimx_ln_qkv_pack": (c_int, [c_void_p, c_int, c_int, c_void_p, c_size_t]),
+    "dimx_op_ln_qkv_packed": (c_int, [c_void_p, c_void_p, c_void_p, c_void_p, c_void_p, c_void_p, c_void_p, c_void_p, c_int, c_int, c_int, c_void_p]),
     "dimx_op_add_slabs_layernorm": (c_int, [c_int, c_void_p, c_void_p, c_int, ctypes.c_long, c_void_p, c_void_p, c_int,
                                             c_int, c_void_p]),
     "dimx_op_chain": (c_int, [c_void_p, c_int, c_void_p, c_void_p, c_void_p, c_int, c_void_p, c_void_p, c_void_p, c_int,
diff --git a/include/dimx.h b/include/dimx.h
--- a/include/dimx.h
+++ b/include/dimx.h
@@ -146,6 +146,7 @@
 int dimx_stream_state(dimx_handle h, int* frames, int* steps, int* open);
 int dimx_stream_set_events(dimx_handle h, void* ev_start, void* ev_encoded, void* ev_appended, void* ev_stepped);
 int dimx_qkv0_table_builds(dimx_handle h);
+int dimx_ln_qkv_launches(dimx_handle h);
 int dimx_kv0_table_generations(dimx_handle h);
 int dimx_sample_head_generations(dimx_handle h);
 int dimx_debug_chain_fault(dimx_handle h, int n_calls);
@@ -273,6 +274,12 @@
 int dimx_mlp_fused_pack(const float* w1_host, const float* b1_host, const float* w2_host, int C, int F, void* out_host, size_t out_bytes);
 int dimx_op_mlp_fused_packed(float* x, const void* packed, const float* b2, const float* ln_g, const float* ln_b, int M, int C, int F,
                              int act, void* stream);
+int dimx_op_ln_qkv(const float* x, const float* w_host, const float* bias, const float* ln_g, const float* ln_b, void* q, void* k, void* v,
+                   int M, int C, int N, void* stream);
+size_t dimx_ln_qkv_packed_bytes(int C, int N);
+int dimx_ln_qkv_pack(const float* w_host, int C, int N, void* out_host, size_t out_bytes);
+int dimx_op_ln_qkv_packed(const float* x, const void* packed, const float* bias, const float* ln_g, const float* ln_b, void* q, void* k,
+                          void* v, int M, int C, int N, void* stream);
 int dimx_op_add_slabs_layernorm(int out_dtype, float* x, const float* slabs, int nslab, long slab_stride, void* y,
                                 const float* gamma, int M, int C, void* stream);
 int dimx_op_chain(const void* A1, int K1, const void* W1, float* x, const float* slabs, int nslab, const float* gamma,
```

After: 1749 clips/s, median of 6. About the same (+0.5%).
